# kngwyu/mujoco-maze

Measured on AMD Instinct MI355X. Metric: env-steps/sec (whole node), AntUMaze-v0, 4096 envs/GPU, higher is better.
Workload: dtype f32; 1 GPU; AntUMaze-v0, 4096 envs/GPU, frame_skip 5 x RK4, random actions uniform in the action box, auto-reset; 100 untimed settle steps + 5 warm-up steps before the timed window; envs_per_gpu=4096, obs_allgather=False, library=mujoco_maze_amd/csrc/libmazestep.so, lanes_per_env=library default, waves_per_block=1, bad_envs=0

## Files before the change

### mujoco_maze_amd/csrc/ant_newton_rows.h

```cpp
#pragma once
#include <type_traits>

#include "ant_dyn.h"
#include "mz_device.h"

namespace rows {

__host__ __device__ __forceinline__ constexpr int pos2dof(int p) { return (p & 3) < 2 ? 6 + 2 * (p >> 2) + (p & 1) : (p < 12 ? 2 * (p >> 2) + (p & 3) - 2 : p); }
__host__ __device__ __forceinline__ constexpr int dof2pos(int d) { return d < 6 ? 4 * (d >> 1) + 2 + (d & 1) : (d < 14 ? 4 * ((d - 6) >> 1) + ((d - 6) & 1) : d); }
static_assert(dof2pos(0) == 2 && dof2pos(5) == 11 && dof2pos(6) == 0 && dof2pos(13) == 13 && pos2dof(7) == 3 && pos2dof(9) == 11 && pos2dof(15) == 15, "row layout");

template <int P>
__device__ __forceinline__ float bcast(float x) {
  return __int_as_float(__builtin_amdgcn_mov_dpp(__float_as_int(x), 0x150 + P, 0xF, 0xF, true));
}
template <int P>
__device__ __forceinline__ int bcast_i(int x) { return __builtin_amdgcn_mov_dpp(x, 0x150 + P, 0xF, 0xF, true); }
__device__ __forceinline__ float rsum(float x) {
#pragma clang fp contract(off)
  x += __int_as_float(__builtin_amdgcn_mov_dpp(__float_as_int(x), 0xB1, 0xF, 0xF, true));
  x += __int_as_float(__builtin_amdgcn_mov_dpp(__float_as_int(x), 0x4E, 0xF, 0xF, true));
  x += __int_as_float(__builtin_amdgcn_mov_dpp(__float_as_int(x), 0x141, 0xF, 0xF, true));
  x += __int_as_float(__builtin_amdgcn_mov_dpp(__float_as_int(x), 0x140, 0xF, 0xF, true));
  return x;
}

#define MZ_DPP_TAIL " row_mask:0xf bank_mask:0xf\n\t"
#define MZ_MV_MUL(acc, k) "v_mul_f32_dpp %" #acc ", %[x], %[a" #k "] row_newbcast:" #k MZ_DPP_TAIL
#define MZ_MV_FMA(acc, k) "v_fmac_f32_dpp %" #acc ", %[x], %[a" #k "] row_newbcast:" #k MZ_DPP_TAIL

#define MZ_R3_OP(d, x, ctrl) "v_add_f32_dpp %[" #d "], %[" #x "], %[" #x "] " ctrl MZ_DPP_TAIL
#define MZ_R3_FIRST(ctrl) MZ_R3_OP(sa, a, ctrl) MZ_R3_OP(sb, b, ctrl) MZ_R3_OP(sc, c, ctrl)
#define MZ_R3_STEP(ctrl) MZ_R3_OP(sa, sa, ctrl) MZ_R3_OP(sb, sb, ctrl) MZ_R3_OP(sc, sc, ctrl)
#define MZ_R3_TREE MZ_R3_FIRST("quad_perm:[1,0,3,2]") MZ_R3_STEP("quad_perm:[2,3,0,1]") MZ_R3_STEP("row_half_mirror") MZ_R3_STEP("row_mirror")
__device__ __forceinline__ void rsum3(float a, float b, float c, float& sa, float& sb, float& sc) {
  asm("s_nop 1\n\t" MZ_R3_TREE : [sa] "=&v"(sa), [sb] "=&v"(sb), [sc] "=&v"(sc) : [a] "v"(a), [b] "v"(b), [c] "v"(c));
}
__device__ __forceinline__ void rsum3_q1(float a, float b, float c, float& sa, float& sb, float& sc, float& qa, float& qb, float& qc) {
  asm("s_nop 1\n\t" MZ_R3_OP(qa, a, "quad_perm:[1,1,1,1]") MZ_R3_OP(qb, b, "quad_perm:[1,1,1,1]") MZ_R3_OP(qc, c, "quad_perm:[1,1,1,1]") MZ_R3_TREE
      : [sa] "=&v"(sa), [sb] "=&v"(sb), [sc] "=&v"(sc), [qa] "=&v"(qa), [qb] "=&v"(qb), [qc] "=&v"(qc) : [a] "v"(a), [b] "v"(b), [c] "v"(c));
}

#define MZ_R2_FIRST(ctrl) "v_add_f32_dpp %0, %2, %2 " ctrl MZ_DPP_TAIL "v_add_f32_dpp %1, %3, %3 " ctrl MZ_DPP_TAIL
#define MZ_R2_STEP(ctrl) "s_nop 0\n\tv_add_f32_dpp %0, %0, %0 " ctrl MZ_DPP_TAIL "v_add_f32_dpp %1, %1, %1 " ctrl MZ_DPP_TAIL
__device__ __forceinline__ void rsum2(float a, float b, float& sa, float& sb) {
  asm("s_nop 1\n\t" MZ_R2_FIRST("quad_perm:[1,0,3,2]") MZ_R2_STEP("quad_perm:[2,3,0,1]") MZ_R2_STEP("row_half_mirror") MZ_R2_STEP("row_mirror")
      : "=&v"(sa), "=&v"(sb) : "v"(a), "v"(b));
}
#define MZ_R3_MUL "v_mul_f32 %[sa], %[a], %[x]\n\tv_mul_f32 %[sb], %[b], %[x]\n\tv_mul_f32 %[sc], %[c], %[x]\n\t"
__device__ __forceinline__ void rsum3_scaled(float a, float b, float c, float x, float& sa, float& sb, float& sc) {
  asm(MZ_R3_MUL MZ_R3_STEP("quad_perm:[1,0,3,2]") MZ_R3_STEP("quad_perm:[2,3,0,1]") MZ_R3_STEP("row_half_mirror") MZ_R3_STEP("row_mirror")
      : [sa] "=&v"(sa), [sb] "=&v"(sb), [sc] "=&v"(sc) : [a] "v"(a), [b] "v"(b), [c] "v"(c), [x] "v"(x));
}

__device__ __forceinline__ float matvec(const float (&A)[14], float x) {
  float s0, s1, s2;
  asm("s_nop 1\n\t" MZ_MV_MUL(0, 0) MZ_MV_MUL(1, 1) MZ_MV_MUL(2, 2) MZ_MV_FMA(0, 3) MZ_MV_FMA(1, 4) MZ_MV_FMA(2, 5) MZ_MV_FMA(0, 6) MZ_MV_FMA(1, 7)
      MZ_MV_FMA(2, 8) MZ_MV_FMA(0, 9) MZ_MV_FMA(1, 10) MZ_MV_FMA(2, 11) MZ_MV_FMA(0, 12) MZ_MV_FMA(1, 13)
      : "=&v"(s0), "=&v"(s1), "=&v"(s2)
      : [x] "v"(x), [a0] "v"(A[0]), [a1] "v"(A[1]), [a2] "v"(A[2]), [a3] "v"(A[3]), [a4] "v"(A[4]), [a5] "v"(A[5]), [a6] "v"(A[6]), [a7] "v"(A[7]),
        [a8] "v"(A[8]), [a9] "v"(A[9]), [a10] "v"(A[10]), [a11] "v"(A[11]), [a12] "v"(A[12]), [a13] "v"(A[13]));
  return (s0 + s1) + s2;
}
__device__ __forceinline__ float matvec(const float (&A)[16], float x) {
  float s0, s1, s2;
  asm("s_nop 1\n\t" MZ_MV_MUL(0, 0) MZ_MV_MUL(1, 1) MZ_MV_MUL(2, 2) MZ_MV_FMA(0, 3) MZ_MV_FMA(1, 4) MZ_MV_FMA(2, 5) MZ_MV_FMA(0, 6) MZ_MV_FMA(1, 7)
      MZ_MV_FMA(2, 8) MZ_MV_FMA(0, 9) MZ_MV_FMA(1, 10) MZ_MV_FMA(2, 11) MZ_MV_FMA(0, 12) MZ_MV_FMA(1, 13) MZ_MV_FMA(2, 14) MZ_MV_FMA(0, 15)
      : "=&v"(s0), "=&v"(s1), "=&v"(s2)
      : [x] "v"(x), [a0] "v"(A[0]), [a1] "v"(A[1]), [a2] "v"(A[2]), [a3] "v"(A[3]), [a4] "v"(A[4]), [a5] "v"(A[5]), [a6] "v"(A[6]), [a7] "v"(A[7]),
        [a8] "v"(A[8]), [a9] "v"(A[9]), [a10] "v"(A[10]), [a11] "v"(A[11]), [a12] "v"(A[12]), [a13] "v"(A[13]), [a14] "v"(A[14]), [a15] "v"(A[15]));
  return (s0 + s1) + s2;
}

#define MZ_EL(i) "v_fmac_f32_dpp %" #i ", %" #i ", %[li] row_newbcast:%[p]" MZ_DPP_TAIL
#define MZ_EL_IN [li] "v"(nli), [p] "n"(P)
template <int P> __device__ __forceinline__ void elim(float nli, float& b) { asm("s_nop 1\n\t" MZ_EL(0) : "+v"(b) : MZ_EL_IN); }
template <int P> __device__ __forceinline__ void elim(float nli, float& b, float& h0) { asm("s_nop 1\n\t" MZ_EL(0) MZ_EL(1) : "+v"(b), "+v"(h0) : MZ_EL_IN); }
template <int P> __device__ __forceinline__ void elim(float nli, float& b, float& h0, float& h1) {
  asm("s_nop 1\n\t" MZ_EL(0) MZ_EL(1) MZ_EL(2) : "+v"(b), "+v"(h0), "+v"(h1) : MZ_EL_IN);
}
template <int P> __device__ __forceinline__ void elim(float nli, float& b, float& h0, float& h1, float& h2) {
  asm("s_nop 1\n\t" MZ_EL(0) MZ_EL(1) MZ_EL(2) MZ_EL(3) : "+v"(b), "+v"(h0), "+v"(h1), "+v"(h2) : MZ_EL_IN);
}
template <int P> __device__ __forceinline__ void elim(float nli, float& b, float& h0, float& h1, float& h2, float& h3) {
  asm("s_nop 1\n\t" MZ_EL(0) MZ_EL(1) MZ_EL(2) MZ_EL(3) MZ_EL(4) : "+v"(b), "+v"(h0), "+v"(h1), "+v"(h2), "+v"(h3) : MZ_EL_IN);
}
template <int P> __device__ __forceinline__ void elim(float nli, float& b, float& h0, float& h1, float& h2, float& h3, float& h4) {
  asm("s_nop 1\n\t" MZ_EL(0) MZ_EL(1) MZ_EL(2) MZ_EL(3) MZ_EL(4) MZ_EL(5) : "+v"(b), "+v"(h0), "+v"(h1), "+v"(h2), "+v"(h3), "+v"(h4) : MZ_EL_IN);
}
template <int P> __device__ __forceinline__ void elim(float nli, float& b, float& h0, float& h1, float& h2, float& h3, float& h4, float& h5) {
  asm("s_nop 1\n\t" MZ_EL(0) MZ_EL(1) MZ_EL(2) MZ_EL(3) MZ_EL(4) MZ_EL(5) MZ_EL(6)
      : "+v"(b), "+v"(h0), "+v"(h1), "+v"(h2), "+v"(h3), "+v"(h4), "+v"(h5) : MZ_EL_IN);
}
template <int P> __device__ __forceinline__ void elim(float nli, float& b, float& h0, float& h1, float& h2, float& h3, float& h4, float& h5, float& h6) {
  asm("s_nop 1\n\t" MZ_EL(0) MZ_EL(1) MZ_EL(2) MZ_EL(3) MZ_EL(4) MZ_EL(5) MZ_EL(6) MZ_EL(7)
      : "+v"(b), "+v"(h0), "+v"(h1), "+v"(h2), "+v"(h3), "+v"(h4), "+v"(h5), "+v"(h6) : MZ_EL_IN);
}
template <int P> __device__ __forceinline__ void elim(float nli, float& b, float& h0, float& h1, float& h2, float& h3, float& h4, float& h5, float& h6, float& h7) {
  asm("s_nop 1\n\t" MZ_EL(0) MZ_EL(1) MZ_EL(2) MZ_EL(3) MZ_EL(4) MZ_EL(5) MZ_EL(6) MZ_EL(7) MZ_EL(8)
      : "+v"(b), "+v"(h0), "+v"(h1), "+v"(h2), "+v"(h3), "+v"(h4), "+v"(h5), "+v"(h6), "+v"(h7) : MZ_EL_IN);
}
template <int P> __device__ __forceinline__ void elim(float nli, float& b, float& h0, float& h1, float& h2, float& h3, float& h4, float& h5, float& h6, float& h7, float& h8) {
  asm("s_nop 1\n\t" MZ_EL(0) MZ_EL(1) MZ_EL(2) MZ_EL(3) MZ_EL(4) MZ_EL(5) MZ_EL(6) MZ_EL(7) MZ_EL(8) MZ_EL(9)
      : "+v"(b), "+v"(h0), "+v"(h1), "+v"(h2), "+v"(h3), "+v"(h4), "+v"(h5), "+v"(h6), "+v"(h7), "+v"(h8) : MZ_EL_IN);
}

#define MZ_FA_MUL(o, c, j) "v_mul_f32_dpp %" #o ", %[" #c "], %[" #j "] row_newbcast:%[p]" MZ_DPP_TAIL
#define MZ_FA_FMA(o, c, j) "v_fmac_f32_dpp %" #o ", %[" #c "], %[" #j "] row_newbcast:%[p]" MZ_DPP_TAIL
template <int P>
__device__ __forceinline__ void fold_t(const float (&cg)[8], float j0, float j1, float j2, float& t, float& t0, float& t1, float& t2) {
  asm("s_nop 1\n\t" MZ_FA_MUL(0, c0, j0) MZ_FA_MUL(1, c3, j0) MZ_FA_MUL(2, c4, j0) MZ_FA_MUL(3, c5, j0) MZ_FA_FMA(0, c1, j1) MZ_FA_FMA(1, c4, j1)
      MZ_FA_FMA(2, c6, j1) MZ_FA_FMA(3, c7, j2) MZ_FA_FMA(0, c2, j2) MZ_FA_FMA(1, c5, j2)
      : "=&v"(t), "=&v"(t0), "=&v"(t1), "=&v"(t2)
      : [c0] "v"(cg[0]), [c1] "v"(cg[1]), [c2] "v"(cg[2]), [c3] "v"(cg[3]), [c4] "v"(cg[4]), [c5] "v"(cg[5]), [c6] "v"(cg[6]), [c7] "v"(cg[7]),
        [j0] "v"(j0), [j1] "v"(j1), [j2] "v"(j2), [p] "n"(P));
}
template <int P>
__device__ __forceinline__ float fold_g(float g0, float g1, float g2, float j0, float j1, float j2) {
  float a0, a1, a2;
  asm("s_nop 1\n\t" MZ_FA_MUL(0, c0, j0) MZ_FA_MUL(1, c1, j1) MZ_FA_MUL(2, c2, j2)
      : "=&v"(a0), "=&v"(a1), "=&v"(a2) : [c0] "v"(g0), [c1] "v"(g1), [c2] "v"(g2), [j0] "v"(j0), [j1] "v"(j1), [j2] "v"(j2), [p] "n"(P));
  return (a0 + a1) + a2;
}
#define MZ_FH(k, j, t) "v_fmac_f32_dpp %" #k ", %[" #j "], %[" #t "] row_newbcast:" #k MZ_DPP_TAIL
#define MZ_FH14(j, t) MZ_FH(0, j, t) MZ_FH(1, j, t) MZ_FH(2, j, t) MZ_FH(3, j, t) MZ_FH(4, j, t) MZ_FH(5, j, t) MZ_FH(6, j, t) MZ_FH(7, j, t) \
                      MZ_FH(8, j, t) MZ_FH(9, j, t) MZ_FH(10, j, t) MZ_FH(11, j, t) MZ_FH(12, j, t) MZ_FH(13, j, t)
#define MZ_FH16(j, t) MZ_FH14(j, t) MZ_FH(14, j, t) MZ_FH(15, j, t)
#define MZ_FH_IN [j0] "v"(j0), [j1] "v"(j1), [j2] "v"(j2), [t0] "v"(t0), [t1] "v"(t1), [t2] "v"(t2)
__device__ __forceinline__ void fold_h(float (&H)[14], float j0, float j1, float j2, float t0, float t1, float t2) {
  asm("s_nop 1\n\t" MZ_FH14(j0, t0) MZ_FH14(j1, t1) MZ_FH14(j2, t2)
      : "+v"(H[0]), "+v"(H[1]), "+v"(H[2]), "+v"(H[3]), "+v"(H[4]), "+v"(H[5]), "+v"(H[6]), "+v"(H[7]), "+v"(H[8]), "+v"(H[9]), "+v"(H[10]),
        "+v"(H[11]), "+v"(H[12]), "+v"(H[13])
      : MZ_FH_IN);
}
__device__ __forceinline__ void fold_h(float (&H)[16], float j0, float j1, float j2, float t0, float t1, float t2) {
  asm("s_nop 1\n\t" MZ_FH16(j0, t0) MZ_FH16(j1, t1) MZ_FH16(j2, t2)
      : "+v"(H[0]), "+v"(H[1]), "+v"(H[2]), "+v"(H[3]), "+v"(H[4]), "+v"(H[5]), "+v"(H[6]), "+v"(H[7]), "+v"(H[8]), "+v"(H[9]), "+v"(H[10]),
        "+v"(H[11]), "+v"(H[12]), "+v"(H[13]), "+v"(H[14]), "+v"(H[15])
      : MZ_FH_IN);
}

typedef float v16f __attribute__((ext_vector_type(16)));
__device__ __forceinline__ void mfma_operands_ready(float& t0, float& t1, float& t2) { asm("s_nop 3" : "+v"(t0), "+v"(t1), "+v"(t2)); }
__device__ __forceinline__ void fold_h_mfma(v16f& acc, float j0, float j1, float j2, float t0, float t1, float t2) {
  mfma_operands_ready(t0, t1, t2);
  acc = __builtin_amdgcn_mfma_f32_16x16x1f32(t0, j0, acc, 0, 0, 0);
  acc = __builtin_amdgcn_mfma_f32_16x16x1f32(t1, j1, acc, 0, 0, 0);
  acc = __builtin_amdgcn_mfma_f32_16x16x1f32(t2, j2, acc, 0, 0, 0);
}
__device__ __forceinline__ void mfma_rows(const v16f& acc, float (&out)[16]) {
  float G[4][4];
#pragma unroll
  for (int b = 0; b < 4; b++)
#pragma unroll
    for (int v = 0; v < 4; v++) G[b][v] = acc[4 * b + v];
#pragma unroll
  for (int v = 0; v < 4; v++) {
    auto r0 = __builtin_amdgcn_permlane32_swap(__float_as_int(G[0][v]), __float_as_int(G[2][v]), false, false);
    G[0][v] = __int_as_float(r0[0]); G[2][v] = __int_as_float(r0[1]);
    auto r1 = __builtin_amdgcn_permlane32_swap(__float_as_int(G[1][v]), __float_as_int(G[3][v]), false, false);
    G[1][v] = __int_as_float(r1[0]); G[3][v] = __int_as_float(r1[1]);
  }
#pragma unroll
  for (int v = 0; v < 4; v++) {
    auto r0 = __builtin_amdgcn_permlane16_swap(__float_as_int(G[0][v]), __float_as_int(G[1][v]), false, false);
    G[0][v] = __int_as_float(r0[0]); G[1][v] = __int_as_float(r0[1]);
    auto r1 = __builtin_amdgcn_permlane16_swap(__float_as_int(G[2][v]), __float_as_int(G[3][v]), false, false);
    G[2][v] = __int_as_float(r1[0]); G[3][v] = __int_as_float(r1[1]);
  }
#pragma unroll
  for (int g = 0; g < 4; g++)
#pragma unroll
    for (int v = 0; v < 4; v++) out[4 * g + v] = G[g][v];
}

__device__ __forceinline__ float pivot_floor() { float t = 1e-30f; asm("" : "+v"(t)); return t; }
template <int P>
__device__ __forceinline__ float pivot_clamped(float h, float tiny) {
  float d;
  asm("s_nop 1\n\tv_max_f32_dpp %0, %1, %2 row_newbcast:%3 row_mask:0xf bank_mask:0xf" : "=&v"(d) : "v"(h), "v"(tiny), "n"(P));
  return d;
}

template <int P, int N, int... COLS>
__device__ __forceinline__ void pivot(int r, float tiny, float (&Hrow)[N], float& b, float& dinv, float (&mlt)[N]) {
  asm("" : "+v"(r));
  const float ri = 1.0f / pivot_clamped<P>(Hrow[P], tiny);
  const float nli = (r == P) ? 0.f : -(Hrow[P] * ri);
  elim<P>(nli, b, Hrow[COLS]...);
  dinv = (r == P) ? ri : dinv;
  mlt[P] = nli;
}

__device__ __forceinline__ float solve_rows(int r, float (&Hrow)[14], float b, float (&mlt)[14], float& dinv) {
  dinv = 0.f;
  const float tiny = pivot_floor();
  pivot<0, 14, 1, 2, 3, 6, 7, 10, 11>(r, tiny, Hrow, b, dinv, mlt);
  pivot<4, 14, 5, 2, 3, 6, 7, 10, 11>(r, tiny, Hrow, b, dinv, mlt);
  pivot<8, 14, 9, 2, 3, 6, 7, 10, 11>(r, tiny, Hrow, b, dinv, mlt);
  pivot<12, 14, 13, 2, 3, 6, 7, 10, 11>(r, tiny, Hrow, b, dinv, mlt);
  pivot<1, 14, 2, 3, 6, 7, 10, 11>(r, tiny, Hrow, b, dinv, mlt);
  pivot<5, 14, 2, 3, 6, 7, 10, 11>(r, tiny, Hrow, b, dinv, mlt);
  pivot<9, 14, 2, 3, 6, 7, 10, 11>(r, tiny, Hrow, b, dinv, mlt);
  pivot<13, 14, 2, 3, 6, 7, 10, 11>(r, tiny, Hrow, b, dinv, mlt);
  pivot<2, 14, 3, 6, 7, 10, 11>(r, tiny, Hrow, b, dinv, mlt);
  pivot<3, 14, 6, 7, 10, 11>(r, tiny, Hrow, b, dinv, mlt);
  pivot<6, 14, 7, 10, 11>(r, tiny, Hrow, b, dinv, mlt);
  pivot<7, 14, 10, 11>(r, tiny, Hrow, b, dinv, mlt);
  pivot<10, 14, 11>(r, tiny, Hrow, b, dinv, mlt);
  pivot<11, 14>(r, tiny, Hrow, b, dinv, mlt);
  return b * dinv;
}
__device__ __forceinline__ float solve_rows(int r, float (&Hrow)[14], float b) {
  float mlt[14], dinv;
  return solve_rows(r, Hrow, b, mlt, dinv);
}
__device__ __forceinline__ float solve_rows(int r, float (&Hrow)[16], float b, float (&mlt)[16], float& dinv) {
  dinv = 0.f;
  const float tiny = pivot_floor();
  pivot<0, 16, 1, 2, 3, 6, 7, 10, 11, 14, 15>(r, tiny, Hrow, b, dinv, mlt);
  pivot<4, 16, 5, 2, 3, 6, 7, 10, 11, 14, 15>(r, tiny, Hrow, b, dinv, mlt);
  pivot<8, 16, 9, 2, 3, 6, 7, 10, 11, 14, 15>(r, tiny, Hrow, b, dinv, mlt);
  pivot<12, 16, 13, 2, 3, 6, 7, 10, 11, 14, 15>(r, tiny, Hrow, b, dinv, mlt);
  pivot<1, 16, 2, 3, 6, 7, 10, 11, 14, 15>(r, tiny, Hrow, b, dinv, mlt);
  pivot<5, 16, 2, 3, 6, 7, 10, 11, 14, 15>(r, tiny, Hrow, b, dinv, mlt);
  pivot<9, 16, 2, 3, 6, 7, 10, 11, 14, 15>(r, tiny, Hrow, b, dinv, mlt);
  pivot<13, 16, 2, 3, 6, 7, 10, 11, 14, 15>(r, tiny, Hrow, b, dinv, mlt);
  pivot<14, 16, 15, 2, 3, 6, 7, 10, 11>(r, tiny, Hrow, b, dinv, mlt);
  pivot<15, 16, 2, 3, 6, 7, 10, 11>(r, tiny, Hrow, b, dinv, mlt);
  pivot<2, 16, 3, 6, 7, 10, 11>(r, tiny, Hrow, b, dinv, mlt);
  pivot<3, 16, 6, 7, 10, 11>(r, tiny, Hrow, b, dinv, mlt);
  pivot<6, 16, 7, 10, 11>(r, tiny, Hrow, b, dinv, mlt);
  pivot<7, 16, 10, 11>(r, tiny, Hrow, b, dinv, mlt);
  pivot<10, 16, 11>(r, tiny, Hrow, b, dinv, mlt);
  pivot<11, 16>(r, tiny, Hrow, b, dinv, mlt);
  return b * dinv;
}

__device__ __forceinline__ float solve_rows(int r, float (&Hrow)[16], float b) {
  float mlt[16], dinv;
  return solve_rows(r, Hrow, b, mlt, dinv);
}
template <int P>
__device__ __forceinline__ void repivot(float m, float& b) { elim<P>(m, b); }
__device__ __forceinline__ float resolve_rows(const float (&mlt)[16], float dinv, float b) {
  repivot<0>(mlt[0], b); repivot<4>(mlt[4], b); repivot<8>(mlt[8], b); repivot<12>(mlt[12], b);
  repivot<1>(mlt[1], b); repivot<5>(mlt[5], b); repivot<9>(mlt[9], b); repivot<13>(mlt[13], b);
  repivot<14>(mlt[14], b); repivot<15>(mlt[15], b);
  repivot<2>(mlt[2], b); repivot<3>(mlt[3], b); repivot<6>(mlt[6], b); repivot<7>(mlt[7], b); repivot<10>(mlt[10], b); repivot<11>(mlt[11], b);
  return b * dinv;
}
__device__ __forceinline__ float resolve_rows(const float (&mlt)[14], float dinv, float b) {
  repivot<0>(mlt[0], b); repivot<4>(mlt[4], b); repivot<8>(mlt[8], b); repivot<12>(mlt[12], b);
  repivot<1>(mlt[1], b); repivot<5>(mlt[5], b); repivot<9>(mlt[9], b); repivot<13>(mlt[13], b);
  repivot<2>(mlt[2], b); repivot<3>(mlt[3], b); repivot<6>(mlt[6], b); repivot<7>(mlt[7], b); repivot<10>(mlt[10], b); repivot<11>(mlt[11], b);
  return b * dinv;
}

#define MZ_D6_MUL(o, k) "v_mul_f32_dpp %" #o ", %[f" #k "], %[s" #k "] row_newbcast:%[q]" MZ_DPP_TAIL
#define MZ_D6_FMA(o, k) "v_fmac_f32_dpp %" #o ", %[f" #k "], %[s" #k "] row_newbcast:%[q]" MZ_DPP_TAIL
template <int Q>
__device__ __forceinline__ float dot6_from(const float (&F)[6], const float (&S)[6]) {
  float a0, a1, a2;
  asm("s_nop 1\n\t" MZ_D6_MUL(0, 0) MZ_D6_MUL(1, 1) MZ_D6_MUL(2, 2) MZ_D6_FMA(0, 3) MZ_D6_FMA(1, 4) MZ_D6_FMA(2, 5)
      : "=&v"(a0), "=&v"(a1), "=&v"(a2)
      : [f0] "v"(F[0]), [f1] "v"(F[1]), [f2] "v"(F[2]), [f3] "v"(F[3]), [f4] "v"(F[4]), [f5] "v"(F[5]), [s0] "v"(S[0]), [s1] "v"(S[1]), [s2] "v"(S[2]),
        [s3] "v"(S[3]), [s4] "v"(S[4]), [s5] "v"(S[5]), [q] "n"(Q));
  return (a0 + a1) + a2;
}
__device__ __forceinline__ float ceval(float D, float u0, float u1, float u2) {
  float r0 = u0 + u1, r1 = u0 - u1, r2 = u0 + u2, r3 = u0 - u2;
  float c = 0.f;
  if (r0 < 0.f) c += r0 * r0;
  if (r1 < 0.f) c += r1 * r1;
  if (r2 < 0.f) c += r2 * r2;
  if (r3 < 0.f) c += r3 * r3;
  return 0.5f * D * c;
}

__device__ __forceinline__ float bsel(int m, float a, float b) { return __int_as_float((__float_as_int(a) & m) | (__float_as_int(b) & ~m)); }

template <int NB>
__device__ __forceinline__ void contact_record(const AntDev& K, const float* pos, const float* n, float dist, int kind, const float* hint, int cls, int leg,
                                               const float* vb, const float* vblk, float tran, float* rec) {
  const int mk = -(int)(kind == 0);
  struct { float margin, mu, K, B; } P = {bsel(mk, K.floor.margin, K.wall.margin), bsel(mk, K.floor.mu, K.wall.mu), bsel(mk, K.floor.K, K.wall.K),
                                         bsel(mk, K.floor.B, K.wall.B)};
  float si[7];
#pragma unroll
  for (int k = 0; k < 7; k++) si[k] = bsel(mk, K.floor.solimp[k], K.wall.solimp[k]);
  float t1[3], t2[3];
  make_tangents(n, hint, t1, t2);
  const float sr = bsel(mk, 1.f, -1.f);
  float omi;
  const float imp = impedance_pair(si, fabsf(dist - P.margin), &omi);
  if (NB == 1 && kind == 2) tran += K.block_bw_tran;
  const float Rr = fmaxf(1e-15f, omi / imp * (tran + P.mu * P.mu * tran));
  rec[7] = 1.0f / (2.f * P.mu * P.mu * Rr);
  rec[15] = __int_as_float((leg < 0 ? 7 : leg) | (cls << 3) | ((NB == 1 && kind == 2) ? 64 : 0));
  rec[23] = 0.f;
#pragma unroll
  for (int a = 0; a < 3; a++) {
    const float sc = (a == 0 ? 1.f : P.mu) * sr;
    const float* dir = a == 0 ? n : (a == 1 ? t1 : t2);
    const float f[3] = {sc * dir[0], sc * dir[1], sc * dir[2]};
    float m[3];
    cross3f(m, pos, f);
    float* w = rec + 8 * a;
    w[0] = m[0]; w[1] = m[1]; w[2] = m[2]; w[3] = f[0]; w[4] = f[1]; w[5] = f[2];
    float vel = m[0] * vb[0] + m[1] * vb[1] + m[2] * vb[2] + f[0] * vb[3] + f[1] * vb[4] + f[2] * vb[5];
    if constexpr (NB == 1) {
      if (kind == 2) {
#pragma unroll
        for (int sl = 0; sl < 2; sl++) vel -= (K.block_axis[sl] == 0 ? f[0] : (K.block_axis[sl] == 1 ? f[1] : f[2])) * vblk[sl];
      }
    }
    float aref = -P.B * vel;
    if (a == 0) aref -= P.K * imp * (dist - P.margin);
    w[6] = aref;
  }
}

__device__ __forceinline__ void contact_raw_store(float* q, const float* pos, const float* n, float dist, int kind, const float* hint, int cls, int leg,
                                                  const float* vb, float tran) {
  float4* dst = reinterpret_cast<float4*>(q);
  dst[0] = make_float4(pos[0], pos[1], pos[2], n[0]);
  dst[1] = make_float4(n[1], n[2], dist, __int_as_float(kind | ((cls + 1) << 4) | ((leg + 1) << 8)));
  dst[2] = make_float4(hint[0], hint[1], hint[2], vb[0]);
  dst[3] = make_float4(vb[1], vb[2], vb[3], vb[4]);
  dst[4] = make_float4(vb[5], tran, 0.f, 0.f);
}
}

template <class S>
__device__ __forceinline__ float* wr_record(S& s, int c) { return &s.cJ[0][0][0] + 24 * c; }
template <class S>
__device__ __forceinline__ const float* wr_record(const S& s, int c) { return &s.cJ[0][0][0] + 24 * c; }

enum { LC_LO = 11, LC_HI = 12, LC_DOFW = 13 };
enum { LU_FLOORM = 14, LU_WALLM, LU_SCALE, LU_INVS, LU_TX, LU_TY, LU_HXY, LU_HZ, LU_CZ, LU_GRID, LU_ARM, LU_DAMP, LU_GZ, LU_TOL, LU_RTOL, LU_ISC,
       LU_ITERS, LU_LS, LU_N };
struct AntU {
  float floor_margin, wall_margin, scale, inv_scale_xy, tx, ty, half_xy, half_z, center_z;
  int rows, cols;
  bool elevated;
  float armature, damping, gz, tol, rtol, inv_scale;
  int max_iter, ls_iter, ls_fast_iters, ls_fast, trust_exact;
};
template <int G, bool PROF>
__device__ __forceinline__ AntU ant_u(const DevCtx<G, PROF>& cx, const AntDev& K) {
  const MazeDev& z = K.maze;
  if (cx.mfma)
    return {K.floor.margin, K.wall.margin, z.scale, 1.0f / z.scale, z.tx, z.ty, z.half_xy, z.half_z, z.center_z, z.rows, z.cols, z.elevated != 0,
            K.armature, K.damping, K.gz, K.tol, K.rtol, K.inv_scale, K.max_iter, K.ls_iter, K.ls_fast_iters, K.ls_fast, K.trust_exact};
  const int g = __float_as_int(cx.lc[LU_GRID]);
  const int a = __builtin_amdgcn_readfirstlane(__float_as_int(cx.lc[LU_ITERS])), b = __builtin_amdgcn_readfirstlane(__float_as_int(cx.lc[LU_LS]));
  return {cx.lc[LU_FLOORM], cx.lc[LU_WALLM], cx.lc[LU_SCALE], cx.lc[LU_INVS], cx.lc[LU_TX], cx.lc[LU_TY], cx.lc[LU_HXY], cx.lc[LU_HZ], cx.lc[LU_CZ],
          g & 255, (g >> 8) & 255, ((g >> 16) & 1) != 0, cx.lc[LU_ARM], cx.lc[LU_DAMP], cx.lc[LU_GZ], cx.lc[LU_TOL], cx.lc[LU_RTOL], cx.lc[LU_ISC],
          a, b & 1023, (b >> 10) & 1023, (b >> 20) & 1023, (b >> 30) & 1};
}
__device__ __forceinline__ float lu_hold(float x) { asm("" : "+v"(x)); return x; }
template <int G, bool PROF>
__device__ __forceinline__ void ant_limit_consts(const AntDev& K, DevCtx<G, PROF>& cx) {
  static_assert(LU_N <= DevCtx<G, PROF>::NLC, "DevCtx::lc too small");
  const int p = cx.l & 15, l = p >> 2, d = p & 1;
  cx.lc[LC_LO] = d ? K.ank_lo[l] : K.hip_lo; cx.lc[LC_HI] = d ? K.ank_hi[l] : K.hip_hi; cx.lc[LC_DOFW] = d ? K.dofw_ank : K.dofw_hip;
  if (cx.mfma) return;
  const MazeDev& z = K.maze;
  cx.lc[LU_FLOORM] = lu_hold(K.floor.margin); cx.lc[LU_WALLM] = lu_hold(K.wall.margin);
  cx.lc[LU_SCALE] = lu_hold(z.scale); cx.lc[LU_INVS] = lu_hold(1.0f / z.scale); cx.lc[LU_TX] = lu_hold(z.tx); cx.lc[LU_TY] = lu_hold(z.ty);
  cx.lc[LU_HXY] = lu_hold(z.half_xy); cx.lc[LU_HZ] = lu_hold(z.half_z); cx.lc[LU_CZ] = lu_hold(z.center_z);
  cx.lc[LU_GRID] = lu_hold(__int_as_float(z.rows | (z.cols << 8) | ((z.elevated ? 1 : 0) << 16)));
  cx.lc[LU_ARM] = lu_hold(K.armature); cx.lc[LU_DAMP] = lu_hold(K.damping); cx.lc[LU_GZ] = lu_hold(K.gz);
  cx.lc[LU_TOL] = lu_hold(K.tol); cx.lc[LU_RTOL] = lu_hold(K.rtol); cx.lc[LU_ISC] = lu_hold(K.inv_scale);
  auto c10 = [](int v) { return v < 0 ? 0 : (v > 1023 ? 1023 : v); };
  cx.lc[LU_ITERS] = lu_hold(__int_as_float(K.max_iter < 0 ? 0 : K.max_iter));
  cx.lc[LU_LS] = lu_hold(__int_as_float(c10(K.ls_iter) | (c10(K.ls_fast_iters) << 10) | (c10(K.ls_fast) << 20) | ((K.trust_exact ? 1 : 0) << 30)));
}

template <int NB>
__device__ __forceinline__ void block_rows_direct(const AntDev& K, const AntScratchCoreT<NB>& s, int c, float (&jb)[3][2], float (&ar)[3], float& Dout) {
  using D = AntDims<NB>;
  const int src = s.csrc[c];
  const float* q = src >= 0 ? con_stage<NB>(s, src) : &s.cY[c][0][0];
  const float n[3] = {q[3], q[4], q[5]}, dist = q[6];
  const int code = (int)q[7], kind = code & 15, other = (code >> 7) & 15;
  const float mult = (float)((code >> 11) + 1);
  const float v0 = s.qvel[14], v1 = s.qvel[15];
  if (kind == 6) {
    const float sg = n[0] + n[1] + n[2];
    jb[0][0] = other == 0 ? sg : 0.f; jb[0][1] = other == 1 ? sg : 0.f;
    jb[1][0] = jb[1][1] = jb[2][0] = jb[2][1] = 0.f;
    const float vel = sg * (other == 0 ? v0 : v1);
    float omi;
    const float imp = impedance_pair(K.blim_solimp, fabsf(dist - K.blim_margin), &omi);
    const float R = fmaxf(1e-15f, omi / imp * K.blim_w);
    Dout = 0.25f / R;
    ar[0] = -K.blim_B * vel - K.blim_K * imp * (dist - K.blim_margin); ar[1] = 0.f; ar[2] = 0.f;
    return;
  }
  const bool fl = kind == 3;
  struct { float margin, mu, K, B; } P = {fl ? K.floor.margin : K.wall.margin, fl ? K.floor.mu : K.wall.mu, fl ? K.floor.K : K.wall.K, fl ? K.floor.B : K.wall.B};
  float psi[7];
#pragma unroll
  for (int k = 0; k < 7; k++) { const float fv = K.floor.solimp[k], wv = K.wall.solimp[k]; psi[k] = fl ? fv : wv; }
  const float hint[3] = {0.f, 0.f, 0.f};
  float t1[3], t2[3];
  make_tangents(n, hint, t1, t2);
#pragma unroll
  for (int a = 0; a < 3; a++) {
    const float sc = a == 0 ? 1.f : P.mu;
    const float* dir = a == 0 ? n : (a == 1 ? t1 : t2);
#pragma unroll
    for (int sl = 0; sl < 2; sl++) jb[a][sl] = sc * (K.block_axis[sl] == 0 ? dir[0] : (K.block_axis[sl] == 1 ? dir[1] : dir[2]));
    ar[a] = -P.B * (jb[a][0] * v0 + jb[a][1] * v1);
  }
  float omi;
  const float imp = impedance_pair(psi, fabsf(dist - P.margin), &omi);
  const float tran = K.block_bw_tran;
  const float R = fmaxf(1e-15f, omi / imp * (tran + P.mu * P.mu * tran));
  Dout = mult / (2.f * P.mu * P.mu * R);
  ar[0] -= P.K * imp * (dist - P.margin);
  (void)sizeof(D);
}

#define MZ_IF_OWNER(c) if (true)
template <int NB, int G, bool PROF, bool WR = false, class SCR>
__device__ __forceinline__ float ant_solve_rows_core(const DevCtx<G, PROF>& cx, const AntDev& K, SCR& s, bool compare,
                                                    const float (&Mrow)[14 + 2 * NB], const float qfs, const float (&Sax)[6], const float hq, const float hv) {
  static_assert(G >= 16, "one DPP row per env at least");
  static_assert(NB <= 1, "one 16-lane row holds 14 dofs + one block's two slides");
  using namespace rows;
  using D = AntDims<NB>;
  constexpr int NR = 14 + 2 * NB;
  constexpr int NHC = D::NH;
  constexpr int BW = WR ? 16 : G;
  constexpr int MB = NB ? (WR ? 1 : (D::NC + G - 1) / G) : 0;
  constexpr int MA = NB ? 2 : 1;
  constexpr bool REFINE = NB == 1;
  const int r = cx.l & 15;
  const bool isdof = r < NR, ishinge = (r & 3) < 2 && r < 14;
  const int leg = r >> 2, d = r & 1;
  const int nB = NB ? s.nblkcon : 0;
  int nA = s.ncon - nB;
  if (nA > 16 * MA) { nA = 16 * MA; if (cx.l == 0) s.status |= MZ_STATUS_CONTACT_OVERFLOW; }
  if (NB && MB * BW < nB && cx.l == 0) s.status |= MZ_STATUS_CONTACT_OVERFLOW;
  auto bsum = [&](float x) { if constexpr (WR) return rsum(x); else return cx.gsum(x); };
  const int ncon = nA;
  const bool any2 = MA > 1 && cx.any(nA > 16);
  bool iscon[MA];
  int cr[MA], cl[MA];
#pragma unroll
  for (int m = 0; m < MA; m++) { iscon[m] = r + 16 * m < ncon; cr[m] = nB + (iscon[m] ? r + 16 * m : 0); cl[m] = (!WR && iscon[m]) ? s.cleg[cr[m]] : -1; }

  const int ri = isdof ? pos2dof(r) : 0;
  cx.tick(s, 12);
  float lsign = 0.f, lD = 0.f, laref = 0.f;
  if (ishinge) {
    const float q = hq, lo = cx.lc[LC_LO], hi = cx.lc[LC_HI];
    float pos = 0.f;
    if (q - lo < 0.f) { lsign = 1.f; pos = q - lo; }
    else if (hi - q < 0.f) { lsign = -1.f; pos = hi - q; }
    if (lsign != 0.f) {
      float omi;
      const float imp = impedance_pair(K.lim_solimp, fabsf(pos), &omi);
      const float R = fmaxf(1e-15f, omi / imp * cx.lc[LC_DOFW]);
      lD = 1.0f / R;
      laref = -K.lim_B * (lsign * hv) - K.lim_K * imp * pos;
    }
  }
  const bool has = s.ncon > 0 || cx.gany(lsign != 0.f);
  float qas = 0.f;
  if (compare || cx.any(!has)) {
    float Hq[NR];
#pragma unroll
    for (int k = 0; k < NR; k++) Hq[k] = Mrow[k];
    qas = solve_rows(r, Hq, qfs);
    if (isdof) s.qas[ri] = qas;
  }
  const float warm = isdof ? s.warm[ri] : 0.f;
  float cD[MA], ar[MA][3];
  float wr[MA][3][6];
  int wmeta[MA];
#pragma unroll
  for (int m = 0; m < MA; m++) wmeta[m] = 0;
  if constexpr (WR) {
#pragma unroll
    for (int m = 0; m < MA; m++) {
#pragma unroll
      for (int a = 0; a < 3; a++) {
#pragma unroll
        for (int k = 0; k < 6; k++) wr[m][a][k] = 0.f;
        ar[m][a] = 0.f;
      }
      cD[m] = 0.f;
      if (m == 1 && !any2) continue;
      const float4* q = reinterpret_cast<const float4*>(wr_record(s, cr[m]));
      float raw[20];
#pragma unroll
      for (int k = 0; k < 5; k++) { const float4 v4 = q[k]; raw[4 * k] = v4.x; raw[4 * k + 1] = v4.y; raw[4 * k + 2] = v4.z; raw[4 * k + 3] = v4.w; }
      const int rmeta = __float_as_int(raw[7]);
      const float vblk[2] = {NB == 1 ? s.qvel[14] : 0.f, NB == 1 ? s.qvel[14 + (NB == 1 ? 1 : 0)] : 0.f};
      float rec[24];
      contact_record<NB>(K, raw, raw + 3, raw[6], rmeta & 15, raw + 8, ((rmeta >> 4) & 15) - 1, ((rmeta >> 8) & 15) - 1, raw + 11, vblk, raw[17], rec);
      const int on = -(int)iscon[m];
#pragma unroll
      for (int a = 0; a < 3; a++) {
#pragma unroll
        for (int k = 0; k < 6; k++) wr[m][a][k] = __int_as_float(__float_as_int(rec[8 * a + k]) & on);
        ar[m][a] = __int_as_float(__float_as_int(rec[8 * a + 6]) & on);
      }
      cD[m] = __int_as_float(__float_as_int(rec[7]) & on);
      wmeta[m] = __float_as_int(rec[15]) & on;
    }
  } else {
#pragma unroll
    for (int m = 0; m < MA; m++) {
      cD[m] = iscon[m] ? s.cD[cr[m]] : 0.f;
#pragma unroll
      for (int a = 0; a < 3; a++) ar[m][a] = iscon[m] ? s.caref[cr[m]][a] : 0.f;
    }
  }
  float bj[MB ? MB : 1][3][2], bar[MB ? MB : 1][3], bD[MB ? MB : 1], bu[MB ? MB : 1][3], bv[MB ? MB : 1][3];
  if constexpr (NB == 1) {
#pragma unroll
    for (int m = 0; m < MB; m++) {
      const int c = (WR ? (cx.l & 15) : cx.l) + m * BW;
      const bool on = c < nB;
      bD[m] = 0.f;
#pragma unroll
      for (int a = 0; a < 3; a++) { bj[m][a][0] = 0.f; bj[m][a][1] = 0.f; bar[m][a] = 0.f; bu[m][a] = 0.f; bv[m][a] = 0.f; }
      if (on) block_rows_direct<NB>(K, s, c, bj[m], bar[m], bD[m]);
    }
  }

  auto each_contact = [&](auto&& f) {
    auto more = [&](int k) { return NB == 1 || cx.any(ncon > k); };
    if (cx.any(ncon > 0)) { f(std::integral_constant<int, 0>{});
    if (more(1)) { f(std::integral_constant<int, 1>{});
    if (more(2)) { f(std::integral_constant<int, 2>{});
    if (more(3)) { f(std::integral_constant<int, 3>{});
      if (cx.any(ncon > 4)) {
        f(std::integral_constant<int, 4>{}); f(std::integral_constant<int, 5>{});
        if (cx.any(ncon > 6)) { f(std::integral_constant<int, 6>{}); f(std::integral_constant<int, 7>{}); }
        if (cx.any(ncon > 8)) {
          f(std::integral_constant<int, 8>{}); f(std::integral_constant<int, 9>{}); f(std::integral_constant<int, 10>{}); f(std::integral_constant<int, 11>{});
          if (cx.any(ncon > 12)) { f(std::integral_constant<int, 12>{}); f(std::integral_constant<int, 13>{}); f(std::integral_constant<int, 14>{}); f(std::integral_constant<int, 15>{}); }
          if constexpr (MA > 1) {
            if (any2) {
              f(std::integral_constant<int, 16>{}); f(std::integral_constant<int, 17>{}); f(std::integral_constant<int, 18>{}); f(std::integral_constant<int, 19>{});
              if (cx.any(ncon > 20)) {
                f(std::integral_constant<int, 20>{}); f(std::integral_constant<int, 21>{}); f(std::integral_constant<int, 22>{}); f(std::integral_constant<int, 23>{});
                if (cx.any(ncon > 24)) {
                  f(std::integral_constant<int, 24>{}); f(std::integral_constant<int, 25>{}); f(std::integral_constant<int, 26>{}); f(std::integral_constant<int, 27>{});
                  f(std::integral_constant<int, 28>{}); f(std::integral_constant<int, 29>{}); f(std::integral_constant<int, 30>{}); f(std::integral_constant<int, 31>{});
                }
              }
            }
          }
        }
      }
    }}}}
  };
  constexpr int NJ = WR ? 16 : 16 * MA;
  float jown[NJ][3];
  auto wr_col = [&](auto Cc, float (&o)[3]) {
    constexpr int C = decltype(Cc)::value;
    const int mc = bcast_i<(C & 15)>(wmeta[C / 16]), lc = mc & 7, cc = (mc >> 3) & 7;
    const bool sees = C < ncon && (ishinge ? (leg == lc && (d == 0 ? cc >= 2 : cc == 3)) : (r < 12 || (NB == 1 && r >= 14 && (mc & 64) != 0)));
    const int on = -(int)sees;
#pragma unroll
    for (int a = 0; a < 3; a++) o[a] = __int_as_float(__float_as_int(dot6_from<(C & 15)>(wr[C / 16][a], Sax)) & on);
  };
  auto own_col = [&](auto Cc, float (&o)[3]) {
    constexpr int C = decltype(Cc)::value;
    if constexpr (WR && C >= 16) wr_col(Cc, o);
    else { o[0] = jown[C < NJ ? C : 0][0]; o[1] = jown[C < NJ ? C : 0][1]; o[2] = jown[C < NJ ? C : 0][2]; }
  };
  each_contact([&](auto Cc) {
    constexpr int C = decltype(Cc)::value;
    if constexpr (WR && C >= 16) return;
    else {
    jown[C][0] = jown[C][1] = jown[C][2] = 0.f;
    if constexpr (WR) {
      wr_col(Cc, jown[C]);
    } else
    if (C < ncon) {
      const int lc = s.cleg[nB + C];
      const int col = ishinge ? (leg == lc ? NHC + d : -1) : (r < 12 ? ri : ((NB == 1 && r >= 14 && r < 16) ? r - 8 : -1));
      if (col >= 0) { jown[C][0] = s.cJ[nB + C][0][col]; jown[C][1] = s.cJ[nB + C][1][col]; jown[C][2] = s.cJ[nB + C][2][col]; }
    }
    }
  });
  float Jf[MA][3][NR];
  if constexpr (!WR)
#pragma unroll
  for (int m = 0; m < MA; m++) {
#pragma unroll
    for (int a = 0; a < 3; a++)
#pragma unroll
      for (int k = 0; k < NR; k++) Jf[m][a][k] = 0.f;
    if (m == 1 && !any2) continue;
    if (iscon[m]) {
#pragma unroll
      for (int a = 0; a < 3; a++) {
        const float* Jr = s.cJ[cr[m]][a];
#pragma unroll
        for (int k = 0; k < 6; k++) Jf[m][a][dof2pos(k)] = Jr[k];
        if constexpr (NB == 1) { Jf[m][a][14] = Jr[6]; Jf[m][a][15] = Jr[7]; }
        const float jh = Jr[NHC], ja = Jr[NHC + 1];
#pragma unroll
        for (int l2 = 0; l2 < 4; l2++) { Jf[m][a][4 * l2] = cl[m] == l2 ? jh : 0.f; Jf[m][a][4 * l2 + 1] = cl[m] == l2 ? ja : 0.f; }
      }
    }
  }
  auto jdot3 = [&](float x, float (&o)[MA][3]) {
    if constexpr (WR) {
#pragma unroll
      for (int m = 0; m < MA; m++) o[m][0] = o[m][1] = o[m][2] = 0.f;
      each_contact([&](auto Cc) {
        constexpr int C = decltype(Cc)::value;
        {
          float jc[3];
          own_col(Cc, jc);
          float t0, t1, t2;
          rsum3_scaled(jc[0], jc[1], jc[2], x, t0, t1, t2);
          if (r == (C & 15)) { o[C / 16][0] = t0; o[C / 16][1] = t1; o[C / 16][2] = t2; }
        }
      });
    } else {
#pragma unroll
      for (int m = 0; m < MA; m++) {
        o[m][0] = o[m][1] = o[m][2] = 0.f;
        if (m == 1 && !any2) continue;
        o[m][0] = matvec(Jf[m][0], x); o[m][1] = matvec(Jf[m][1], x); o[m][2] = matvec(Jf[m][2], x);
      }
    }
  };
  auto bdot = [&](float b0, float b1, float (&o)[MB ? MB : 1][3]) {
#pragma unroll
    for (int m = 0; m < MB; m++)
#pragma unroll
      for (int a = 0; a < 3; a++) o[m][a] = bj[m][a][0] * b0 + bj[m][a][1] * b1;
  };

  float qacc = warm;
  if (compare) {
    const float dw = warm - qas;
    float cw = 0.5f * dw * matvec(Mrow, dw), cs = 0.f;
    float jw3[MA][3], jq3[MA][3];
    jdot3(warm, jw3);
    jdot3(qas, jq3);
#pragma unroll
    for (int m = 0; m < MA; m++)
      if (iscon[m]) {
        cw += ceval(cD[m], jw3[m][0] - ar[m][0], jw3[m][1] - ar[m][1], jw3[m][2] - ar[m][2]);
        cs += ceval(cD[m], jq3[m][0] - ar[m][0], jq3[m][1] - ar[m][1], jq3[m][2] - ar[m][2]);
      }
    if (lsign != 0.f) {
      const float jw = lsign * warm - laref, js = lsign * qas - laref;
      if (jw < 0.f) cw += 0.5f * lD * jw * jw;
      if (js < 0.f) cs += 0.5f * lD * js * js;
    }
    rsum2(cw, cs, cw, cs);
    if constexpr (NB == 1) {
      float bw[MB][3], bs[MB][3], cwb = 0.f, csb = 0.f;
      bdot(bcast<14>(warm), bcast<15>(warm), bw);
      bdot(bcast<14>(qas), bcast<15>(qas), bs);
#pragma unroll
      for (int m = 0; m < MB; m++) {
        cwb += ceval(bD[m], bw[m][0] - bar[m][0], bw[m][1] - bar[m][1], bw[m][2] - bar[m][2]);
        csb += ceval(bD[m], bs[m][0] - bar[m][0], bs[m][1] - bar[m][1], bs[m][2] - bar[m][2]);
      }
      cw += bsum(cwb); cs += bsum(csb);
    }
    qacc = cw < cs ? warm : qas;
  }
  if (!has) qacc = qas;
  cx.tick(s, 4);
  bool done = !has;
  int it = 0;
  float Mx = 0.f, ljar = 0.f, lact = 0.f, u[MA][3], v[MA][3];
#pragma unroll
  for (int m = 0; m < MA; m++) { u[m][0] = u[m][1] = u[m][2] = 0.f; v[m][0] = v[m][1] = v[m][2] = 0.f; }
  if (cx.any(!done)) {
    Mx = matvec(Mrow, qacc) - qfs;
    jdot3(qacc, u);
#pragma unroll
    for (int m = 0; m < MA; m++) { u[m][0] -= ar[m][0]; u[m][1] -= ar[m][1]; u[m][2] -= ar[m][2]; }
    if (lsign != 0.f) { ljar = lsign * qacc - laref; lact = ljar < 0.f ? lD : 0.f; }
    if constexpr (NB == 1) {
      bdot(bcast<14>(qacc), bcast<15>(qacc), bu);
#pragma unroll
      for (int m = 0; m < MB; m++)
#pragma unroll
        for (int a = 0; a < 3; a++) bu[m][a] -= bar[m][a];
    }
  }
  while (cx.any(!done) && it < ant_u(cx, K).max_iter) {
    float mycg[MA][8];
#pragma unroll
    for (int m = 0; m < MA; m++) {
#pragma unroll
      for (int k = 0; k < 8; k++) mycg[m][k] = 0.f;
      if (m == 1 && !any2) continue;
      MZ_IF_OWNER(iscon[m]) {
        const float u0 = u[m][0], u1 = u[m][1], u2 = u[m][2], Dm = cD[m];
        const float r0 = u0 + u1, r1 = u0 - u1, r2 = u0 + u2, r3 = u0 - u2;
        const float a0 = r0 < 0.f ? 1.f : 0.f, a1 = r1 < 0.f ? 1.f : 0.f, a2 = r2 < 0.f ? 1.f : 0.f, a3 = r3 < 0.f ? 1.f : 0.f;
        mycg[m][0] = Dm * (a0 * r0 + a1 * r1 + a2 * r2 + a3 * r3); mycg[m][1] = Dm * (a0 * r0 - a1 * r1); mycg[m][2] = Dm * (a2 * r2 - a3 * r3);
        mycg[m][3] = Dm * (a0 + a1 + a2 + a3); mycg[m][4] = Dm * (a0 - a1); mycg[m][5] = Dm * (a2 - a3); mycg[m][6] = Dm * (a0 + a1); mycg[m][7] = Dm * (a2 + a3);
      }
    }
    float bg0 = 0.f, bg1 = 0.f, bga0 = 0.f, bga1 = 0.f, bh00 = 0.f, bh01 = 0.f, bh11 = 0.f;
    if constexpr (NB == 1) {
#pragma unroll
      for (int m = 0; m < MB; m++) {
        const float x0 = bu[m][0], x1 = bu[m][1], x2 = bu[m][2], Dm = bD[m];
        const float r0 = x0 + x1, r1 = x0 - x1, r2 = x0 + x2, r3 = x0 - x2;
        const float a0 = r0 < 0.f ? 1.f : 0.f, a1 = r1 < 0.f ? 1.f : 0.f, a2 = r2 < 0.f ? 1.f : 0.f, a3 = r3 < 0.f ? 1.f : 0.f;
        const float g0 = Dm * (a0 * r0 + a1 * r1 + a2 * r2 + a3 * r3), g1 = Dm * (a0 * r0 - a1 * r1), g2 = Dm * (a2 * r2 - a3 * r3);
        const float W0 = Dm * (a0 + a1 + a2 + a3), W1 = Dm * (a0 - a1), W2 = Dm * (a2 - a3), W3 = Dm * (a0 + a1), W4 = Dm * (a2 + a3);
#pragma unroll
        for (int c = 0; c < 2; c++) {
          const float j0 = bj[m][0][c], j1 = bj[m][1][c], j2 = bj[m][2][c];
          const float t = j0 * g0 + j1 * g1 + j2 * g2;
          if (c == 0) { bg0 += t; bga0 += fabsf(t); } else { bg1 += t; bga1 += fabsf(t); }
          const float t0 = j0 * W0 + j1 * W1 + j2 * W2, t1 = j0 * W1 + j1 * W3, t2 = j0 * W2 + j2 * W4;
          if (c == 0) { bh00 += t0 * j0 + t1 * j1 + t2 * j2; bh01 += t0 * bj[m][0][1] + t1 * bj[m][1][1] + t2 * bj[m][2][1]; }
          else bh11 += t0 * j0 + t1 * j1 + t2 * j2;
        }
      }
      if constexpr (WR) {
        rsum3(bg0, bg1, bh00, bg0, bg1, bh00); rsum2(bga0, bga1, bga0, bga1); rsum2(bh01, bh11, bh01, bh11);
      } else {
        bg0 = bsum(bg0); bg1 = bsum(bg1); bga0 = bsum(bga0); bga1 = bsum(bga1);
        bh00 = bsum(bh00); bh01 = bsum(bh01); bh11 = bsum(bh11);
      }
    }
    float Hrow[NR];
#pragma unroll
    for (int k = 0; k < NR; k++) Hrow[k] = Mrow[k];
    float g = Mx, ga = fabsf(Mx);
    if (cx.mfma) {
     if (cx.any(ncon > 0)) {
      v16f hacc = {0.f, 0.f, 0.f, 0.f, 0.f, 0.f, 0.f, 0.f, 0.f, 0.f, 0.f, 0.f, 0.f, 0.f, 0.f, 0.f};
      each_contact([&](auto Cc) {
        constexpr int C = decltype(Cc)::value;
        float t, t0, t1, t2;
        float jc[3];
        own_col(Cc, jc);
        fold_t<(C & 15)>(mycg[C / 16], jc[0], jc[1], jc[2], t, t0, t1, t2);
        g += t; ga += fabsf(t);
        fold_h_mfma(hacc, jc[0], jc[1], jc[2], t0, t1, t2);
      });
      float hc[16];
      mfma_rows(hacc, hc);
#pragma unroll
      for (int k = 0; k < NR; k++) Hrow[k] += hc[k];
     }
    } else
    each_contact([&](auto Cc) {
      constexpr int C = decltype(Cc)::value;
      {
        float t, t0, t1, t2;
        float jc[3];
        own_col(Cc, jc);
        fold_t<(C & 15)>(mycg[C / 16], jc[0], jc[1], jc[2], t, t0, t1, t2);
        g += t; ga += fabsf(t);
        fold_h(Hrow, jc[0], jc[1], jc[2], t0, t1, t2);
      }
    });
    if constexpr (NB == 1) {
      if (r == 14) { g += bg0; ga += bga0; Hrow[14] += bh00; Hrow[15] += bh01; }
      if (r == 15) { g += bg1; ga += bga1; Hrow[14] += bh01; Hrow[15] += bh11; }
    }
    MZ_IF_OWNER(lsign != 0.f) { const float t = lsign * lact * ljar; g += t; ga += fabsf(t); }
#pragma unroll
    for (int k = 0; k < 14; k++)
      if ((k & 3) < 2) Hrow[k] += (r == k) ? lact : 0.f;
    if (!isdof) { g = 0.f; ga = 0.f; }
    float gnorm = 0.f, anorm = 0.f;
    if (it > 0) {
      rsum2(g * g, ga * ga, gnorm, anorm);
      gnorm = sqrtf(gnorm); anorm = sqrtf(anorm);
      if (!done && (ant_u(cx, K).inv_scale * gnorm < ant_u(cx, K).tol || gnorm <= ant_u(cx, K).rtol * anorm)) done = true;
    }
    if (!cx.any(!done)) { cx.tick(s, 5); break; }
    cx.tick(s, 5);
    float mlt[NR], dinv;
    const float search = solve_rows(r, Hrow, -g, mlt, dinv);
    cx.tick(s, 6);
    jdot3(search, v);
    const float ljv = lsign * search;
    bool changed = false;
#pragma unroll
    for (int m = 0; m < MA; m++)
      if (m == 0 || any2) MZ_IF_OWNER(iscon[m]) {
        const float u0 = u[m][0], u1 = u[m][1], u2 = u[m][2], w0 = u0 + v[m][0], w1 = u1 + v[m][1], w2 = u2 + v[m][2];
        changed = changed || ((u0 + u1 < 0.f) != (w0 + w1 < 0.f)) || ((u0 - u1 < 0.f) != (w0 - w1 < 0.f)) || ((u0 + u2 < 0.f) != (w0 + w2 < 0.f)) ||
                  ((u0 - u2 < 0.f) != (w0 - w2 < 0.f));
      }
    MZ_IF_OWNER(lsign != 0.f) changed = changed || ((ljar < 0.f) != (ljar + ljv < 0.f));
    if constexpr (NB == 1) {
      bdot(bcast<14>(search), bcast<15>(search), bv);
#pragma unroll
      for (int m = 0; m < MB; m++) {
        const float x0 = bu[m][0], x1 = bu[m][1], x2 = bu[m][2], w0 = x0 + bv[m][0], w1 = x1 + bv[m][1], w2 = x2 + bv[m][2];
        changed = changed || ((x0 + x1 < 0.f) != (w0 + w1 < 0.f)) || ((x0 - x1 < 0.f) != (w0 - w1 < 0.f)) || ((x0 + x2 < 0.f) != (w0 + w2 < 0.f)) ||
                  ((x0 - x2 < 0.f) != (w0 - w2 < 0.f));
      }
    }
    changed = cx.gany(changed);
    float alpha = 1.f, Ms = 0.f, sn = 1.f, qn = 0.f;
    const bool exact = !changed;
    if (changed) {
      Ms = matvec(Mrow, search);
      float p1, p2;
      rsum2(search * Mx, search * Ms, p1, p2);
      rsum2(isdof ? search * search : 0.f, isdof ? qacc * qacc : 0.f, sn, qn);
      float lo = 0.f, hi = -1.f, prev_d2 = -1.f;
      const int ls_max = it < ant_u(cx, K).ls_fast_iters ? ant_u(cx, K).ls_fast : ant_u(cx, K).ls_iter;
      for (int ls = 0; ls < ls_max; ls++) {
        float d1 = 0.f, d2 = 0.f;
#pragma unroll
        for (int m = 0; m < MA; m++)
          if (m == 0 || any2) MZ_IF_OWNER(iscon[m]) {
            const float v0 = v[m][0], v1 = v[m][1], v2 = v[m][2], Dm = cD[m];
            const float x0 = u[m][0] + alpha * v0, x1 = u[m][1] + alpha * v1, x2 = u[m][2] + alpha * v2;
            float rr, vv;
            rr = x0 + x1; vv = v0 + v1; if (rr < 0.f) { d1 += Dm * rr * vv; d2 += Dm * vv * vv; }
            rr = x0 - x1; vv = v0 - v1; if (rr < 0.f) { d1 += Dm * rr * vv; d2 += Dm * vv * vv; }
            rr = x0 + x2; vv = v0 + v2; if (rr < 0.f) { d1 += Dm * rr * vv; d2 += Dm * vv * vv; }
            rr = x0 - x2; vv = v0 - v2; if (rr < 0.f) { d1 += Dm * rr * vv; d2 += Dm * vv * vv; }
          }
        MZ_IF_OWNER(lsign != 0.f) { const float rr = ljar + alpha * ljv; if (rr < 0.f) { d1 += lD * rr * ljv; d2 += lD * ljv * ljv; } }
        if constexpr (NB != 1 || !WR) {
          rsum2(d1, d2, d1, d2);
          d1 = d1 + p1 + alpha * p2;
          d2 = d2 + p2;
        }
        if constexpr (NB == 1) {
          float e1 = 0.f, e2 = 0.f;
#pragma unroll
          for (int m = 0; m < MB; m++) {
            const float y0 = bv[m][0], y1 = bv[m][1], y2 = bv[m][2], Dm = bD[m];
            const float x0 = bu[m][0] + alpha * y0, x1 = bu[m][1] + alpha * y1, x2 = bu[m][2] + alpha * y2;
            float rr, vv;
            rr = x0 + x1; vv = y0 + y1; if (rr < 0.f) { e1 += Dm * rr * vv; e2 += Dm * vv * vv; }
            rr = x0 - x1; vv = y0 - y1; if (rr < 0.f) { e1 += Dm * rr * vv; e2 += Dm * vv * vv; }
            rr = x0 + x2; vv = y0 + y2; if (rr < 0.f) { e1 += Dm * rr * vv; e2 += Dm * vv * vv; }
            rr = x0 - x2; vv = y0 - y2; if (rr < 0.f) { e1 += Dm * rr * vv; e2 += Dm * vv * vv; }
          }
          if constexpr (WR) { rsum2(d1 + e1, d2 + e2, d1, d2); d1 = d1 + p1 + alpha * p2; d2 = d2 + p2; }
          else { d1 += cx.gsum(e1); d2 += cx.gsum(e2); }
        }
        if (d2 == prev_d2) break;
        prev_d2 = d2;
        if (d1 < 0.f) lo = alpha; else hi = alpha;
        float next = alpha - d1 / d2;
        if (hi >= 0.f && !(next > lo && next < hi)) next = 0.5f * (lo + hi);
        if (!(next > 0.f)) next = hi >= 0.f ? 0.5f * (lo + hi) : 0.f;
        if (fabsf(next - alpha) <= 1e-7f * fabsf(next)) { alpha = next; break; }
        alpha = next;
      }
    }
    if (done) alpha = 0.f;
    if (alpha != 0.f) {
      qacc += alpha * search;
      if (changed) {
        Mx += alpha * Ms;
#pragma unroll
        for (int m = 0; m < MA; m++) { u[m][0] += alpha * v[m][0]; u[m][1] += alpha * v[m][1]; u[m][2] += alpha * v[m][2]; }
        MZ_IF_OWNER(lsign != 0.f) { ljar += alpha * ljv; lact = ljar < 0.f ? lD : 0.f; }
        if constexpr (NB == 1) {
#pragma unroll
          for (int m = 0; m < MB; m++)
#pragma unroll
            for (int a = 0; a < 3; a++) bu[m][a] += alpha * bv[m][a];
        }
      }
    }
    if constexpr (REFINE) {
      if (cx.any(exact && !done)) {
        const float Ms2 = changed ? Ms : matvec(Mrow, search);
        float g2 = Mx + Ms2;
        float cg2[MA][3];
#pragma unroll
        for (int m = 0; m < MA; m++) {
          cg2[m][0] = cg2[m][1] = cg2[m][2] = 0.f;
          if (m == 1 && !any2) continue;
          const float u0 = u[m][0] + v[m][0], u1 = u[m][1] + v[m][1], u2 = u[m][2] + v[m][2], Dm = cD[m];
          const float r0 = u0 + u1, r1 = u0 - u1, r2 = u0 + u2, r3 = u0 - u2;
          const float a0 = r0 < 0.f ? r0 : 0.f, a1 = r1 < 0.f ? r1 : 0.f, a2 = r2 < 0.f ? r2 : 0.f, a3 = r3 < 0.f ? r3 : 0.f;
          cg2[m][0] = Dm * (a0 + a1 + a2 + a3); cg2[m][1] = Dm * (a0 - a1); cg2[m][2] = Dm * (a2 - a3);
        }
        each_contact([&](auto Cc) {
          constexpr int C = decltype(Cc)::value;
          float jc[3];
          own_col(Cc, jc);
          g2 += fold_g<(C & 15)>(cg2[C / 16][0], cg2[C / 16][1], cg2[C / 16][2], jc[0], jc[1], jc[2]);
        });
        {
          const float lj2 = ljar + ljv;
          g2 += lsign * (lj2 < 0.f ? lD : 0.f) * lj2;
        }
        if constexpr (NB == 1) {
          float c0 = 0.f, c1 = 0.f;
#pragma unroll
          for (int m = 0; m < MB; m++) {
            const float x0 = bu[m][0] + bv[m][0], x1 = bu[m][1] + bv[m][1], x2 = bu[m][2] + bv[m][2], Dm = bD[m];
            const float r0 = x0 + x1, r1 = x0 - x1, r2 = x0 + x2, r3 = x0 - x2;
            const float a0 = r0 < 0.f ? r0 : 0.f, a1 = r1 < 0.f ? r1 : 0.f, a2 = r2 < 0.f ? r2 : 0.f, a3 = r3 < 0.f ? r3 : 0.f;
            const float g0 = Dm * (a0 + a1 + a2 + a3), g1 = Dm * (a0 - a1), gg2 = Dm * (a2 - a3);
            c0 += bj[m][0][0] * g0 + bj[m][1][0] * g1 + bj[m][2][0] * gg2;
            c1 += bj[m][0][1] * g0 + bj[m][1][1] * g1 + bj[m][2][1] * gg2;
          }
          if constexpr (WR) rsum2(c0, c1, c0, c1); else { c0 = bsum(c0); c1 = bsum(c1); }
          if (r == 14) g2 += c0;
          if (r == 15) g2 += c1;
        }
        if (!isdof) g2 = 0.f;
        const float corr = resolve_rows(mlt, dinv, -g2);
        if (exact && !done) qacc += corr;
      }
    }
    if (exact && ant_u(cx, K).trust_exact) done = true;
    if (changed && alpha * alpha * sn <= MZ_NEWTON_STALL * MZ_NEWTON_STALL * qn) done = true;
    cx.tick(s, 7);
    it++;
  }
  if (isdof) s.qacc[ri] = qacc;
  if (cx.l == 0) {
    s.iters = it;
    if (it >= ant_u(cx, K).max_iter && !done) s.status |= MZ_STATUS_SOLVER_MAXITER;
    if constexpr (PROF) s.prof[15] += (unsigned)it;
  }
  cx.sync();
  cx.tick(s, 8);
  return qacc;
}
```

Measured before the change: 18.07 million env-steps/s.

## Fuse Newton solver DPP asm blocks and do Gauss-Jordan elimination in place

Rewrites the row-parallel Newton solver's hand-written DPP assembly. Hessian fold_t and fold_h are merged into one asm block. The pivot chain becomes a single in-place Gauss-Jordan asm sequence that keeps the multipliers in Hrow instead of a separate mlt array. Two rsum2 reductions are merged into one rsum4, and the three dot6 calls into one dot6x3. The aim is to cut s_nop wait states, asm boundaries and register pressure, at the cost of fragile hand-scheduled hazard handling and reuse of Hrow as multiplier storage.

After: 18.80 million env-steps/s, median of 6. 1.04x the previous value.

```diff
diff --git a/mujoco_maze_amd/csrc/ant_newton_rows.h b/mujoco_maze_amd/csrc/ant_newton_rows.h
--- a/mujoco_maze_amd/csrc/ant_newton_rows.h
+++ b/mujoco_maze_amd/csrc/ant_newton_rows.h
@@ -26,6 +26,13 @@
 }
 
 #define MZ_DPP_TAIL " row_mask:0xf bank_mask:0xf\n\t"
+#define MZ_ASM_W(W, body, ...)                                       \
+  do {                                                               \
+    static_assert(W >= 0 && W <= 2, "opening wait states: 0, 1, 2"); \
+    if constexpr (W == 0) asm(body __VA_ARGS__);                     \
+    else if constexpr (W == 1) asm("s_nop 0\n\t" body __VA_ARGS__);  \
+    else asm("s_nop 1\n\t" body __VA_ARGS__);                        \
+  } while (0)
 #define MZ_MV_MUL(acc, k) "v_mul_f32_dpp %" #acc ", %[x], %[a" #k "] row_newbcast:" #k MZ_DPP_TAIL
 #define MZ_MV_FMA(acc, k) "v_fmac_f32_dpp %" #acc ", %[x], %[a" #k "] row_newbcast:" #k MZ_DPP_TAIL
 
@@ -33,19 +40,34 @@
 #define MZ_R3_FIRST(ctrl) MZ_R3_OP(sa, a, ctrl) MZ_R3_OP(sb, b, ctrl) MZ_R3_OP(sc, c, ctrl)
 #define MZ_R3_STEP(ctrl) MZ_R3_OP(sa, sa, ctrl) MZ_R3_OP(sb, sb, ctrl) MZ_R3_OP(sc, sc, ctrl)
 #define MZ_R3_TREE MZ_R3_FIRST("quad_perm:[1,0,3,2]") MZ_R3_STEP("quad_perm:[2,3,0,1]") MZ_R3_STEP("row_half_mirror") MZ_R3_STEP("row_mirror")
+template <int W = 2>
 __device__ __forceinline__ void rsum3(float a, float b, float c, float& sa, float& sb, float& sc) {
-  asm("s_nop 1\n\t" MZ_R3_TREE : [sa] "=&v"(sa), [sb] "=&v"(sb), [sc] "=&v"(sc) : [a] "v"(a), [b] "v"(b), [c] "v"(c));
-}
+  MZ_ASM_W(W, MZ_R3_TREE, : [sa] "=&v"(sa), [sb] "=&v"(sb), [sc] "=&v"(sc) : [a] "v"(a), [b] "v"(b), [c] "v"(c));
+}
+template <int W = 2>
 __device__ __forceinline__ void rsum3_q1(float a, float b, float c, float& sa, float& sb, float& sc, float& qa, float& qb, float& qc) {
-  asm("s_nop 1\n\t" MZ_R3_OP(qa, a, "quad_perm:[1,1,1,1]") MZ_R3_OP(qb, b, "quad_perm:[1,1,1,1]") MZ_R3_OP(qc, c, "quad_perm:[1,1,1,1]") MZ_R3_TREE
-      : [sa] "=&v"(sa), [sb] "=&v"(sb), [sc] "=&v"(sc), [qa] "=&v"(qa), [qb] "=&v"(qb), [qc] "=&v"(qc) : [a] "v"(a), [b] "v"(b), [c] "v"(c));
+  MZ_ASM_W(W, MZ_R3_OP(qa, a, "quad_perm:[1,1,1,1]") MZ_R3_OP(qb, b, "quad_perm:[1,1,1,1]") MZ_R3_OP(qc, c, "quad_perm:[1,1,1,1]") MZ_R3_TREE,
+           : [sa] "=&v"(sa), [sb] "=&v"(sb), [sc] "=&v"(sc), [qa] "=&v"(qa), [qb] "=&v"(qb), [qc] "=&v"(qc) : [a] "v"(a), [b] "v"(b), [c] "v"(c));
 }
 
 #define MZ_R2_FIRST(ctrl) "v_add_f32_dpp %0, %2, %2 " ctrl MZ_DPP_TAIL "v_add_f32_dpp %1, %3, %3 " ctrl MZ_DPP_TAIL
 #define MZ_R2_STEP(ctrl) "s_nop 0\n\tv_add_f32_dpp %0, %0, %0 " ctrl MZ_DPP_TAIL "v_add_f32_dpp %1, %1, %1 " ctrl MZ_DPP_TAIL
+template <int W = 2>
 __device__ __forceinline__ void rsum2(float a, float b, float& sa, float& sb) {
-  asm("s_nop 1\n\t" MZ_R2_FIRST("quad_perm:[1,0,3,2]") MZ_R2_STEP("quad_perm:[2,3,0,1]") MZ_R2_STEP("row_half_mirror") MZ_R2_STEP("row_mirror")
+  MZ_ASM_W(W, MZ_R2_FIRST("quad_perm:[1,0,3,2]") MZ_R2_STEP("quad_perm:[2,3,0,1]") MZ_R2_STEP("row_half_mirror") MZ_R2_STEP("row_mirror"),
+           : "=&v"(sa), "=&v"(sb) : "v"(a), "v"(b));
+}
+__device__ __forceinline__ void rsum2_sq(float a, float b, float& sa, float& sb) {
+  asm("v_mul_f32 %0, %2, %2\n\tv_mul_f32 %1, %3, %3\n\t" MZ_R2_STEP("quad_perm:[1,0,3,2]") MZ_R2_STEP("quad_perm:[2,3,0,1]") MZ_R2_STEP("row_half_mirror")
+      MZ_R2_STEP("row_mirror")
       : "=&v"(sa), "=&v"(sb) : "v"(a), "v"(b));
+}
+#define MZ_R4_FIRST(ctrl) MZ_R3_FIRST(ctrl) MZ_R3_OP(sd, d, ctrl)
+#define MZ_R4_STEP(ctrl) MZ_R3_STEP(ctrl) MZ_R3_OP(sd, sd, ctrl)
+template <int W = 2>
+__device__ __forceinline__ void rsum4(float a, float b, float c, float d, float& sa, float& sb, float& sc, float& sd) {
+  MZ_ASM_W(W, MZ_R4_FIRST("quad_perm:[1,0,3,2]") MZ_R4_STEP("quad_perm:[2,3,0,1]") MZ_R4_STEP("row_half_mirror") MZ_R4_STEP("row_mirror"),
+           : [sa] "=&v"(sa), [sb] "=&v"(sb), [sc] "=&v"(sc), [sd] "=&v"(sd) : [a] "v"(a), [b] "v"(b), [c] "v"(c), [d] "v"(d));
 }
 #define MZ_R3_MUL "v_mul_f32 %[sa], %[a], %[x]\n\tv_mul_f32 %[sb], %[b], %[x]\n\tv_mul_f32 %[sc], %[c], %[x]\n\t"
 __device__ __forceinline__ void rsum3_scaled(float a, float b, float c, float x, float& sa, float& sb, float& sc) {
@@ -53,91 +75,65 @@
       : [sa] "=&v"(sa), [sb] "=&v"(sb), [sc] "=&v"(sc) : [a] "v"(a), [b] "v"(b), [c] "v"(c), [x] "v"(x));
 }
 
+template <int W = 2>
 __device__ __forceinline__ float matvec(const float (&A)[14], float x) {
   float s0, s1, s2;
-  asm("s_nop 1\n\t" MZ_MV_MUL(0, 0) MZ_MV_MUL(1, 1) MZ_MV_MUL(2, 2) MZ_MV_FMA(0, 3) MZ_MV_FMA(1, 4) MZ_MV_FMA(2, 5) MZ_MV_FMA(0, 6) MZ_MV_FMA(1, 7)
-      MZ_MV_FMA(2, 8) MZ_MV_FMA(0, 9) MZ_MV_FMA(1, 10) MZ_MV_FMA(2, 11) MZ_MV_FMA(0, 12) MZ_MV_FMA(1, 13)
+  MZ_ASM_W(W, MZ_MV_MUL(0, 0) MZ_MV_MUL(1, 1) MZ_MV_MUL(2, 2) MZ_MV_FMA(0, 3) MZ_MV_FMA(1, 4) MZ_MV_FMA(2, 5) MZ_MV_FMA(0, 6) MZ_MV_FMA(1, 7)
+      MZ_MV_FMA(2, 8) MZ_MV_FMA(0, 9) MZ_MV_FMA(1, 10) MZ_MV_FMA(2, 11) MZ_MV_FMA(0, 12) MZ_MV_FMA(1, 13),
       : "=&v"(s0), "=&v"(s1), "=&v"(s2)
       : [x] "v"(x), [a0] "v"(A[0]), [a1] "v"(A[1]), [a2] "v"(A[2]), [a3] "v"(A[3]), [a4] "v"(A[4]), [a5] "v"(A[5]), [a6] "v"(A[6]), [a7] "v"(A[7]),
         [a8] "v"(A[8]), [a9] "v"(A[9]), [a10] "v"(A[10]), [a11] "v"(A[11]), [a12] "v"(A[12]), [a13] "v"(A[13]));
   return (s0 + s1) + s2;
 }
+template <int W = 2>
 __device__ __forceinline__ float matvec(const float (&A)[16], float x) {
   float s0, s1, s2;
-  asm("s_nop 1\n\t" MZ_MV_MUL(0, 0) MZ_MV_MUL(1, 1) MZ_MV_MUL(2, 2) MZ_MV_FMA(0, 3) MZ_MV_FMA(1, 4) MZ_MV_FMA(2, 5) MZ_MV_FMA(0, 6) MZ_MV_FMA(1, 7)
-      MZ_MV_FMA(2, 8) MZ_MV_FMA(0, 9) MZ_MV_FMA(1, 10) MZ_MV_FMA(2, 11) MZ_MV_FMA(0, 12) MZ_MV_FMA(1, 13) MZ_MV_FMA(2, 14) MZ_MV_FMA(0, 15)
+  MZ_ASM_W(W, MZ_MV_MUL(0, 0) MZ_MV_MUL(1, 1) MZ_MV_MUL(2, 2) MZ_MV_FMA(0, 3) MZ_MV_FMA(1, 4) MZ_MV_FMA(2, 5) MZ_MV_FMA(0, 6) MZ_MV_FMA(1, 7)
+      MZ_MV_FMA(2, 8) MZ_MV_FMA(0, 9) MZ_MV_FMA(1, 10) MZ_MV_FMA(2, 11) MZ_MV_FMA(0, 12) MZ_MV_FMA(1, 13) MZ_MV_FMA(2, 14) MZ_MV_FMA(0, 15),
       : "=&v"(s0), "=&v"(s1), "=&v"(s2)
       : [x] "v"(x), [a0] "v"(A[0]), [a1] "v"(A[1]), [a2] "v"(A[2]), [a3] "v"(A[3]), [a4] "v"(A[4]), [a5] "v"(A[5]), [a6] "v"(A[6]), [a7] "v"(A[7]),
         [a8] "v"(A[8]), [a9] "v"(A[9]), [a10] "v"(A[10]), [a11] "v"(A[11]), [a12] "v"(A[12]), [a13] "v"(A[13]), [a14] "v"(A[14]), [a15] "v"(A[15]));
   return (s0 + s1) + s2;
 }
 
-#define MZ_EL(i) "v_fmac_f32_dpp %" #i ", %" #i ", %[li] row_newbcast:%[p]" MZ_DPP_TAIL
-#define MZ_EL_IN [li] "v"(nli), [p] "n"(P)
-template <int P> __device__ __forceinline__ void elim(float nli, float& b) { asm("s_nop 1\n\t" MZ_EL(0) : "+v"(b) : MZ_EL_IN); }
-template <int P> __device__ __forceinline__ void elim(float nli, float& b, float& h0) { asm("s_nop 1\n\t" MZ_EL(0) MZ_EL(1) : "+v"(b), "+v"(h0) : MZ_EL_IN); }
-template <int P> __device__ __forceinline__ void elim(float nli, float& b, float& h0, float& h1) {
-  asm("s_nop 1\n\t" MZ_EL(0) MZ_EL(1) MZ_EL(2) : "+v"(b), "+v"(h0), "+v"(h1) : MZ_EL_IN);
-}
-template <int P> __device__ __forceinline__ void elim(float nli, float& b, float& h0, float& h1, float& h2) {
-  asm("s_nop 1\n\t" MZ_EL(0) MZ_EL(1) MZ_EL(2) MZ_EL(3) : "+v"(b), "+v"(h0), "+v"(h1), "+v"(h2) : MZ_EL_IN);
-}
-template <int P> __device__ __forceinline__ void elim(float nli, float& b, float& h0, float& h1, float& h2, float& h3) {
-  asm("s_nop 1\n\t" MZ_EL(0) MZ_EL(1) MZ_EL(2) MZ_EL(3) MZ_EL(4) : "+v"(b), "+v"(h0), "+v"(h1), "+v"(h2), "+v"(h3) : MZ_EL_IN);
-}
-template <int P> __device__ __forceinline__ void elim(float nli, float& b, float& h0, float& h1, float& h2, float& h3, float& h4) {
-  asm("s_nop 1\n\t" MZ_EL(0) MZ_EL(1) MZ_EL(2) MZ_EL(3) MZ_EL(4) MZ_EL(5) : "+v"(b), "+v"(h0), "+v"(h1), "+v"(h2), "+v"(h3), "+v"(h4) : MZ_EL_IN);
-}
-template <int P> __device__ __forceinline__ void elim(float nli, float& b, float& h0, float& h1, float& h2, float& h3, float& h4, float& h5) {
-  asm("s_nop 1\n\t" MZ_EL(0) MZ_EL(1) MZ_EL(2) MZ_EL(3) MZ_EL(4) MZ_EL(5) MZ_EL(6)
-      : "+v"(b), "+v"(h0), "+v"(h1), "+v"(h2), "+v"(h3), "+v"(h4), "+v"(h5) : MZ_EL_IN);
-}
-template <int P> __device__ __forceinline__ void elim(float nli, float& b, float& h0, float& h1, float& h2, float& h3, float& h4, float& h5, float& h6) {
-  asm("s_nop 1\n\t" MZ_EL(0) MZ_EL(1) MZ_EL(2) MZ_EL(3) MZ_EL(4) MZ_EL(5) MZ_EL(6) MZ_EL(7)
-      : "+v"(b), "+v"(h0), "+v"(h1), "+v"(h2), "+v"(h3), "+v"(h4), "+v"(h5), "+v"(h6) : MZ_EL_IN);
-}
-template <int P> __device__ __forceinline__ void elim(float nli, float& b, float& h0, float& h1, float& h2, float& h3, float& h4, float& h5, float& h6, float& h7) {
-  asm("s_nop 1\n\t" MZ_EL(0) MZ_EL(1) MZ_EL(2) MZ_EL(3) MZ_EL(4) MZ_EL(5) MZ_EL(6) MZ_EL(7) MZ_EL(8)
-      : "+v"(b), "+v"(h0), "+v"(h1), "+v"(h2), "+v"(h3), "+v"(h4), "+v"(h5), "+v"(h6), "+v"(h7) : MZ_EL_IN);
-}
-template <int P> __device__ __forceinline__ void elim(float nli, float& b, float& h0, float& h1, float& h2, float& h3, float& h4, float& h5, float& h6, float& h7, float& h8) {
-  asm("s_nop 1\n\t" MZ_EL(0) MZ_EL(1) MZ_EL(2) MZ_EL(3) MZ_EL(4) MZ_EL(5) MZ_EL(6) MZ_EL(7) MZ_EL(8) MZ_EL(9)
-      : "+v"(b), "+v"(h0), "+v"(h1), "+v"(h2), "+v"(h3), "+v"(h4), "+v"(h5), "+v"(h6), "+v"(h7), "+v"(h8) : MZ_EL_IN);
-}
 
 #define MZ_FA_MUL(o, c, j) "v_mul_f32_dpp %" #o ", %[" #c "], %[" #j "] row_newbcast:%[p]" MZ_DPP_TAIL
 #define MZ_FA_FMA(o, c, j) "v_fmac_f32_dpp %" #o ", %[" #c "], %[" #j "] row_newbcast:%[p]" MZ_DPP_TAIL
-template <int P>
+#define MZ_FT(t, t0, t1, t2)                                                                                                        \
+  MZ_FA_MUL(t0, c3, j0) MZ_FA_MUL(t, c0, j0) MZ_FA_MUL(t1, c4, j0) MZ_FA_FMA(t0, c4, j1) MZ_FA_FMA(t, c1, j1) MZ_FA_MUL(t2, c5, j0) \
+  MZ_FA_FMA(t0, c5, j2) MZ_FA_FMA(t, c2, j2) MZ_FA_FMA(t1, c6, j1) MZ_FA_FMA(t2, c7, j2)
+#define MZ_FT_IN                                                                                                                             \
+  [c0] "v"(cg[0]), [c1] "v"(cg[1]), [c2] "v"(cg[2]), [c3] "v"(cg[3]), [c4] "v"(cg[4]), [c5] "v"(cg[5]), [c6] "v"(cg[6]), [c7] "v"(cg[7]), \
+      [j0] "v"(j0), [j1] "v"(j1), [j2] "v"(j2), [p] "n"(P)
+template <int P, int W = 2>
 __device__ __forceinline__ void fold_t(const float (&cg)[8], float j0, float j1, float j2, float& t, float& t0, float& t1, float& t2) {
-  asm("s_nop 1\n\t" MZ_FA_MUL(0, c0, j0) MZ_FA_MUL(1, c3, j0) MZ_FA_MUL(2, c4, j0) MZ_FA_MUL(3, c5, j0) MZ_FA_FMA(0, c1, j1) MZ_FA_FMA(1, c4, j1)
-      MZ_FA_FMA(2, c6, j1) MZ_FA_FMA(3, c7, j2) MZ_FA_FMA(0, c2, j2) MZ_FA_FMA(1, c5, j2)
-      : "=&v"(t), "=&v"(t0), "=&v"(t1), "=&v"(t2)
-      : [c0] "v"(cg[0]), [c1] "v"(cg[1]), [c2] "v"(cg[2]), [c3] "v"(cg[3]), [c4] "v"(cg[4]), [c5] "v"(cg[5]), [c6] "v"(cg[6]), [c7] "v"(cg[7]),
-        [j0] "v"(j0), [j1] "v"(j1), [j2] "v"(j2), [p] "n"(P));
-}
-template <int P>
+  MZ_ASM_W(W, MZ_FT(0, 1, 2, 3), : "=&v"(t), "=&v"(t0), "=&v"(t1), "=&v"(t2) : MZ_FT_IN);
+}
+template <int P, int W = 2>
 __device__ __forceinline__ float fold_g(float g0, float g1, float g2, float j0, float j1, float j2) {
   float a0, a1, a2;
-  asm("s_nop 1\n\t" MZ_FA_MUL(0, c0, j0) MZ_FA_MUL(1, c1, j1) MZ_FA_MUL(2, c2, j2)
+  MZ_ASM_W(W, MZ_FA_MUL(0, c0, j0) MZ_FA_MUL(1, c1, j1) MZ_FA_MUL(2, c2, j2),
       : "=&v"(a0), "=&v"(a1), "=&v"(a2) : [c0] "v"(g0), [c1] "v"(g1), [c2] "v"(g2), [j0] "v"(j0), [j1] "v"(j1), [j2] "v"(j2), [p] "n"(P));
   return (a0 + a1) + a2;
 }
-#define MZ_FH(k, j, t) "v_fmac_f32_dpp %" #k ", %[" #j "], %[" #t "] row_newbcast:" #k MZ_DPP_TAIL
-#define MZ_FH14(j, t) MZ_FH(0, j, t) MZ_FH(1, j, t) MZ_FH(2, j, t) MZ_FH(3, j, t) MZ_FH(4, j, t) MZ_FH(5, j, t) MZ_FH(6, j, t) MZ_FH(7, j, t) \
-                      MZ_FH(8, j, t) MZ_FH(9, j, t) MZ_FH(10, j, t) MZ_FH(11, j, t) MZ_FH(12, j, t) MZ_FH(13, j, t)
-#define MZ_FH16(j, t) MZ_FH14(j, t) MZ_FH(14, j, t) MZ_FH(15, j, t)
-#define MZ_FH_IN [j0] "v"(j0), [j1] "v"(j1), [j2] "v"(j2), [t0] "v"(t0), [t1] "v"(t1), [t2] "v"(t2)
-__device__ __forceinline__ void fold_h(float (&H)[14], float j0, float j1, float j2, float t0, float t1, float t2) {
-  asm("s_nop 1\n\t" MZ_FH14(j0, t0) MZ_FH14(j1, t1) MZ_FH14(j2, t2)
-      : "+v"(H[0]), "+v"(H[1]), "+v"(H[2]), "+v"(H[3]), "+v"(H[4]), "+v"(H[5]), "+v"(H[6]), "+v"(H[7]), "+v"(H[8]), "+v"(H[9]), "+v"(H[10]),
-        "+v"(H[11]), "+v"(H[12]), "+v"(H[13])
-      : MZ_FH_IN);
-}
-__device__ __forceinline__ void fold_h(float (&H)[16], float j0, float j1, float j2, float t0, float t1, float t2) {
-  asm("s_nop 1\n\t" MZ_FH16(j0, t0) MZ_FH16(j1, t1) MZ_FH16(j2, t2)
-      : "+v"(H[0]), "+v"(H[1]), "+v"(H[2]), "+v"(H[3]), "+v"(H[4]), "+v"(H[5]), "+v"(H[6]), "+v"(H[7]), "+v"(H[8]), "+v"(H[9]), "+v"(H[10]),
-        "+v"(H[11]), "+v"(H[12]), "+v"(H[13]), "+v"(H[14]), "+v"(H[15])
-      : MZ_FH_IN);
+#define MZ_FTH(k, j, t) "v_fmac_f32_dpp %[h" #k "], %[" #j "], %[" #t "] row_newbcast:" #k MZ_DPP_TAIL
+#define MZ_FTH14(j, t) MZ_FTH(0, j, t) MZ_FTH(1, j, t) MZ_FTH(2, j, t) MZ_FTH(3, j, t) MZ_FTH(4, j, t) MZ_FTH(5, j, t) MZ_FTH(6, j, t) MZ_FTH(7, j, t) \
+                       MZ_FTH(8, j, t) MZ_FTH(9, j, t) MZ_FTH(10, j, t) MZ_FTH(11, j, t) MZ_FTH(12, j, t) MZ_FTH(13, j, t)
+#define MZ_FTH16(j, t) MZ_FTH14(j, t) MZ_FTH(14, j, t) MZ_FTH(15, j, t)
+#define MZ_FTH_OUT14                                                                                                                              \
+  [t] "=&v"(t), [t0] "=&v"(t0), [t1] "=&v"(t1), [t2] "=&v"(t2), [h0] "+v"(H[0]), [h1] "+v"(H[1]), [h2] "+v"(H[2]), [h3] "+v"(H[3]), [h4] "+v"(H[4]), \
+      [h5] "+v"(H[5]), [h6] "+v"(H[6]), [h7] "+v"(H[7]), [h8] "+v"(H[8]), [h9] "+v"(H[9]), [h10] "+v"(H[10]), [h11] "+v"(H[11]), [h12] "+v"(H[12]), [h13] "+v"(H[13])
+template <int P, int W = 2>
+__device__ __forceinline__ float fold_th(float (&H)[14], const float (&cg)[8], float j0, float j1, float j2) {
+  float t, t0, t1, t2;
+  MZ_ASM_W(W, MZ_FT([t], [t0], [t1], [t2]) MZ_FTH14(j0, t0) MZ_FTH14(j1, t1) MZ_FTH14(j2, t2), : MZ_FTH_OUT14 : MZ_FT_IN);
+  return t;
+}
+template <int P, int W = 2>
+__device__ __forceinline__ float fold_th(float (&H)[16], const float (&cg)[8], float j0, float j1, float j2) {
+  float t, t0, t1, t2;
+  MZ_ASM_W(W, MZ_FT([t], [t0], [t1], [t2]) MZ_FTH16(j0, t0) MZ_FTH16(j1, t1) MZ_FTH16(j2, t2), : MZ_FTH_OUT14, [h14] "+v"(H[14]), [h15] "+v"(H[15]) : MZ_FT_IN);
+  return t;
 }
 
 typedef float v16f __attribute__((ext_vector_type(16)));
@@ -174,99 +170,123 @@
     for (int v = 0; v < 4; v++) out[4 * g + v] = G[g][v];
 }
 
-__device__ __forceinline__ float pivot_floor() { float t = 1e-30f; asm("" : "+v"(t)); return t; }
-template <int P>
-__device__ __forceinline__ float pivot_clamped(float h, float tiny) {
-  float d;
-  asm("s_nop 1\n\tv_max_f32_dpp %0, %1, %2 row_newbcast:%3 row_mask:0xf bank_mask:0xf" : "=&v"(d) : "v"(h), "v"(tiny), "n"(P));
-  return d;
-}
-
-template <int P, int N, int... COLS>
-__device__ __forceinline__ void pivot(int r, float tiny, float (&Hrow)[N], float& b, float& dinv, float (&mlt)[N]) {
-  asm("" : "+v"(r));
-  const float ri = 1.0f / pivot_clamped<P>(Hrow[P], tiny);
-  const float nli = (r == P) ? 0.f : -(Hrow[P] * ri);
-  elim<P>(nli, b, Hrow[COLS]...);
-  dinv = (r == P) ? ri : dinv;
-  mlt[P] = nli;
-}
-
-__device__ __forceinline__ float solve_rows(int r, float (&Hrow)[14], float b, float (&mlt)[14], float& dinv) {
+typedef unsigned long long lanemask_t;
+#define MZ_GJ_CMP(m, p) "v_cmp_eq_u32_e64 %[" #m "], " #p ", %[r]\n\t"
+#define MZ_GJ_GAP "s_nop 0\n\t"
+#define MZ_GJ_B(p) "v_fmac_f32_dpp %[b], %[b], %[h" #p "] row_newbcast:" #p MZ_DPP_TAIL
+#define MZ_GJ_E(k, p) "v_fmac_f32_dpp %[h" #k "], %[h" #k "], %[h" #p "] row_newbcast:" #p MZ_DPP_TAIL
+#define MZ_GJ_PIVOT(p, m, slot, el)                                                      \
+  "v_max_f32_dpp %[ri], %[h" #p "], %[tiny] row_newbcast:" #p MZ_DPP_TAIL                \
+  "v_rcp_f32_e32 %[ri], %[ri]\n\t" slot "v_mul_f32_e64 %[h" #p "], %[h" #p "], -%[ri]\n\t" \
+  "v_cndmask_b32_e64 %[h" #p "], %[h" #p "], 0, %[" #m "]\n\t"                             \
+  "v_cndmask_b32_e64 %[dinv], %[dinv], %[ri], %[" #m "]\n\t"                               \
+  "s_nop 0\n\t" el
+#define MZ_GJ_HINGE(p, pn, rk, rn, el)                                                                                    \
+  MZ_GJ_CMP(mb, p) "v_mul_f32_e64 %[h" #p "], %[h" #p "], -%[" #rk "]\n\t"                                                 \
+  "v_max_f32_dpp %[" #rn "], %[h" #pn "], %[tiny] row_newbcast:" #pn MZ_DPP_TAIL "v_cndmask_b32_e64 %[h" #p "], %[h" #p "], 0, %[mb]\n\t" \
+  "v_rcp_f32_e32 %[" #rn "], %[" #rn "]\n\t" "v_cndmask_b32_e64 %[dinv], %[dinv], %[" #rk "], %[mb]\n\t" el
+#define MZ_GJ_HINGE13(pn, el)                                                                                           \
+  MZ_GJ_CMP(mb, 13) "v_mul_f32_e64 %[h13], %[h13], -%[rj]\n\t" MZ_GJ_CMP(ma, pn) "v_cndmask_b32_e64 %[h13], %[h13], 0, %[mb]\n\t" \
+  "v_cndmask_b32_e64 %[dinv], %[dinv], %[rj], %[mb]\n\t" "s_nop 0\n\t" el
+#define MZ_GJ_OPEN "s_nop 1\n\tv_max_f32_dpp %[ri], %[h0], %[tiny] row_newbcast:0" MZ_DPP_TAIL "v_rcp_f32_e32 %[ri], %[ri]\n\t"
+#define MZ_GJ_ROOT(p) MZ_GJ_E(2, p) MZ_GJ_E(3, p) MZ_GJ_E(6, p) MZ_GJ_E(7, p) MZ_GJ_E(10, p) MZ_GJ_E(11, p)
+#define MZ_GJ_TAIL                                                           \
+  MZ_GJ_PIVOT(2, ma, MZ_GJ_CMP(mb, 3), MZ_GJ_B(2) MZ_GJ_E(3, 2) MZ_GJ_E(6, 2) MZ_GJ_E(7, 2) MZ_GJ_E(10, 2) MZ_GJ_E(11, 2))                      \
+  MZ_GJ_PIVOT(3, mb, MZ_GJ_CMP(ma, 6), MZ_GJ_B(3) MZ_GJ_E(6, 3) MZ_GJ_E(7, 3) MZ_GJ_E(10, 3) MZ_GJ_E(11, 3))                                   \
+  MZ_GJ_PIVOT(6, ma, MZ_GJ_CMP(mb, 7), MZ_GJ_B(6) MZ_GJ_E(7, 6) MZ_GJ_E(10, 6) MZ_GJ_E(11, 6))                                                \
+  MZ_GJ_PIVOT(7, mb, MZ_GJ_CMP(ma, 10), MZ_GJ_B(7) MZ_GJ_E(10, 7) MZ_GJ_E(11, 7))                                                             \
+  "s_nop 0\n\t" MZ_GJ_PIVOT(10, ma, MZ_GJ_CMP(mb, 11), MZ_GJ_B(10) MZ_GJ_E(11, 10)) "s_nop 1\n\t" MZ_GJ_PIVOT(11, mb, MZ_GJ_GAP, MZ_GJ_B(11))
+#define MZ_GJ_OPS14                                                                                                                          \
+  [b] "+v"(b), [dinv] "+v"(dinv), [h0] "+v"(H[0]), [h1] "+v"(H[1]), [h2] "+v"(H[2]), [h3] "+v"(H[3]), [h4] "+v"(H[4]), [h5] "+v"(H[5]),        \
+      [h6] "+v"(H[6]), [h7] "+v"(H[7]), [h8] "+v"(H[8]), [h9] "+v"(H[9]), [h10] "+v"(H[10]), [h11] "+v"(H[11]), [h12] "+v"(H[12]), [h13] "+v"(H[13])
+#define MZ_GJ_TMP [ri] "=&v"(ri), [rj] "=&v"(rj), [ma] "=&s"(ma), [mb] "=&s"(mb) : [tiny] "v"(tiny), [r] "v"(r)
+__device__ __forceinline__ float solve_rows(int r, float (&H)[14], float b, float& dinv) {
   dinv = 0.f;
-  const float tiny = pivot_floor();
-  pivot<0, 14, 1, 2, 3, 6, 7, 10, 11>(r, tiny, Hrow, b, dinv, mlt);
-  pivot<4, 14, 5, 2, 3, 6, 7, 10, 11>(r, tiny, Hrow, b, dinv, mlt);
-  pivot<8, 14, 9, 2, 3, 6, 7, 10, 11>(r, tiny, Hrow, b, dinv, mlt);
-  pivot<12, 14, 13, 2, 3, 6, 7, 10, 11>(r, tiny, Hrow, b, dinv, mlt);
-  pivot<1, 14, 2, 3, 6, 7, 10, 11>(r, tiny, Hrow, b, dinv, mlt);
-  pivot<5, 14, 2, 3, 6, 7, 10, 11>(r, tiny, Hrow, b, dinv, mlt);
-  pivot<9, 14, 2, 3, 6, 7, 10, 11>(r, tiny, Hrow, b, dinv, mlt);
-  pivot<13, 14, 2, 3, 6, 7, 10, 11>(r, tiny, Hrow, b, dinv, mlt);
-  pivot<2, 14, 3, 6, 7, 10, 11>(r, tiny, Hrow, b, dinv, mlt);
-  pivot<3, 14, 6, 7, 10, 11>(r, tiny, Hrow, b, dinv, mlt);
-  pivot<6, 14, 7, 10, 11>(r, tiny, Hrow, b, dinv, mlt);
-  pivot<7, 14, 10, 11>(r, tiny, Hrow, b, dinv, mlt);
-  pivot<10, 14, 11>(r, tiny, Hrow, b, dinv, mlt);
-  pivot<11, 14>(r, tiny, Hrow, b, dinv, mlt);
+  float tiny = 1e-30f, ri, rj;
+  asm("" : "+v"(tiny));
+  lanemask_t ma, mb;
+  asm(MZ_GJ_OPEN
+      MZ_GJ_HINGE(0, 4, ri, rj, MZ_GJ_B(0) MZ_GJ_E(1, 0) MZ_GJ_ROOT(0))
+      MZ_GJ_HINGE(4, 8, rj, ri, MZ_GJ_B(4) MZ_GJ_E(5, 4) MZ_GJ_ROOT(4))
+      MZ_GJ_HINGE(8, 12, ri, rj, MZ_GJ_B(8) MZ_GJ_E(9, 8) MZ_GJ_ROOT(8))
+      MZ_GJ_HINGE(12, 1, rj, ri, MZ_GJ_B(12) MZ_GJ_E(13, 12) MZ_GJ_ROOT(12))
+      MZ_GJ_HINGE(1, 5, ri, rj, MZ_GJ_B(1) MZ_GJ_ROOT(1))
+      MZ_GJ_HINGE(5, 9, rj, ri, MZ_GJ_B(5) MZ_GJ_ROOT(5))
+      MZ_GJ_HINGE(9, 13, ri, rj, MZ_GJ_B(9) MZ_GJ_ROOT(9))
+      MZ_GJ_HINGE13(2, MZ_GJ_B(13) MZ_GJ_ROOT(13))
+      MZ_GJ_TAIL
+      : MZ_GJ_OPS14, MZ_GJ_TMP);
   return b * dinv;
 }
 __device__ __forceinline__ float solve_rows(int r, float (&Hrow)[14], float b) {
-  float mlt[14], dinv;
-  return solve_rows(r, Hrow, b, mlt, dinv);
-}
-__device__ __forceinline__ float solve_rows(int r, float (&Hrow)[16], float b, float (&mlt)[16], float& dinv) {
+  float dinv;
+  return solve_rows(r, Hrow, b, dinv);
+}
+#define MZ_GJ_HUB16(p) MZ_GJ_ROOT(p) MZ_GJ_E(14, p) MZ_GJ_E(15, p)
+__device__ __forceinline__ float solve_rows(int r, float (&H)[16], float b, float& dinv) {
   dinv = 0.f;
-  const float tiny = pivot_floor();
-  pivot<0, 16, 1, 2, 3, 6, 7, 10, 11, 14, 15>(r, tiny, Hrow, b, dinv, mlt);
-  pivot<4, 16, 5, 2, 3, 6, 7, 10, 11, 14, 15>(r, tiny, Hrow, b, dinv, mlt);
-  pivot<8, 16, 9, 2, 3, 6, 7, 10, 11, 14, 15>(r, tiny, Hrow, b, dinv, mlt);
-  pivot<12, 16, 13, 2, 3, 6, 7, 10, 11, 14, 15>(r, tiny, Hrow, b, dinv, mlt);
-  pivot<1, 16, 2, 3, 6, 7, 10, 11, 14, 15>(r, tiny, Hrow, b, dinv, mlt);
-  pivot<5, 16, 2, 3, 6, 7, 10, 11, 14, 15>(r, tiny, Hrow, b, dinv, mlt);
-  pivot<9, 16, 2, 3, 6, 7, 10, 11, 14, 15>(r, tiny, Hrow, b, dinv, mlt);
-  pivot<13, 16, 2, 3, 6, 7, 10, 11, 14, 15>(r, tiny, Hrow, b, dinv, mlt);
-  pivot<14, 16, 15, 2, 3, 6, 7, 10, 11>(r, tiny, Hrow, b, dinv, mlt);
-  pivot<15, 16, 2, 3, 6, 7, 10, 11>(r, tiny, Hrow, b, dinv, mlt);
-  pivot<2, 16, 3, 6, 7, 10, 11>(r, tiny, Hrow, b, dinv, mlt);
-  pivot<3, 16, 6, 7, 10, 11>(r, tiny, Hrow, b, dinv, mlt);
-  pivot<6, 16, 7, 10, 11>(r, tiny, Hrow, b, dinv, mlt);
-  pivot<7, 16, 10, 11>(r, tiny, Hrow, b, dinv, mlt);
-  pivot<10, 16, 11>(r, tiny, Hrow, b, dinv, mlt);
-  pivot<11, 16>(r, tiny, Hrow, b, dinv, mlt);
+  float tiny = 1e-30f, ri, rj;
+  asm("" : "+v"(tiny));
+  lanemask_t ma, mb;
+  asm(MZ_GJ_OPEN
+      MZ_GJ_HINGE(0, 4, ri, rj, MZ_GJ_B(0) MZ_GJ_E(1, 0) MZ_GJ_HUB16(0))
+      MZ_GJ_HINGE(4, 8, rj, ri, MZ_GJ_B(4) MZ_GJ_E(5, 4) MZ_GJ_HUB16(4))
+      MZ_GJ_HINGE(8, 12, ri, rj, MZ_GJ_B(8) MZ_GJ_E(9, 8) MZ_GJ_HUB16(8))
+      MZ_GJ_HINGE(12, 1, rj, ri, MZ_GJ_B(12) MZ_GJ_E(13, 12) MZ_GJ_HUB16(12))
+      MZ_GJ_HINGE(1, 5, ri, rj, MZ_GJ_B(1) MZ_GJ_HUB16(1))
+      MZ_GJ_HINGE(5, 9, rj, ri, MZ_GJ_B(5) MZ_GJ_HUB16(5))
+      MZ_GJ_HINGE(9, 13, ri, rj, MZ_GJ_B(9) MZ_GJ_HUB16(9))
+      MZ_GJ_HINGE13(14, MZ_GJ_B(13) MZ_GJ_HUB16(13))
+      "s_nop 0\n\t" MZ_GJ_PIVOT(14, ma, MZ_GJ_CMP(mb, 15), MZ_GJ_B(14) MZ_GJ_E(15, 14) MZ_GJ_ROOT(14))
+      MZ_GJ_PIVOT(15, mb, MZ_GJ_CMP(ma, 2), MZ_GJ_B(15) MZ_GJ_ROOT(15))
+      MZ_GJ_TAIL
+      : MZ_GJ_OPS14, [h14] "+v"(H[14]), [h15] "+v"(H[15]), MZ_GJ_TMP);
   return b * dinv;
 }
-
 __device__ __forceinline__ float solve_rows(int r, float (&Hrow)[16], float b) {
-  float mlt[16], dinv;
-  return solve_rows(r, Hrow, b, mlt, dinv);
-}
-template <int P>
-__device__ __forceinline__ void repivot(float m, float& b) { elim<P>(m, b); }
+  float dinv;
+  return solve_rows(r, Hrow, b, dinv);
+}
+#define MZ_RP(p) "s_nop 1\n\tv_fmac_f32_dpp %[b], %[b], %[h" #p "] row_newbcast:" #p MZ_DPP_TAIL
+#define MZ_RP_LEGS MZ_RP(0) MZ_RP(4) MZ_RP(8) MZ_RP(12) MZ_RP(1) MZ_RP(5) MZ_RP(9) MZ_RP(13)
+#define MZ_RP_ROOT MZ_RP(2) MZ_RP(3) MZ_RP(6) MZ_RP(7) MZ_RP(10) MZ_RP(11)
+#define MZ_RP_IN14                                                                                                                              \
+  [h0] "v"(mlt[0]), [h1] "v"(mlt[1]), [h2] "v"(mlt[2]), [h3] "v"(mlt[3]), [h4] "v"(mlt[4]), [h5] "v"(mlt[5]), [h6] "v"(mlt[6]), [h7] "v"(mlt[7]), \
+      [h8] "v"(mlt[8]), [h9] "v"(mlt[9]), [h10] "v"(mlt[10]), [h11] "v"(mlt[11]), [h12] "v"(mlt[12]), [h13] "v"(mlt[13])
 __device__ __forceinline__ float resolve_rows(const float (&mlt)[16], float dinv, float b) {
-  repivot<0>(mlt[0], b); repivot<4>(mlt[4], b); repivot<8>(mlt[8], b); repivot<12>(mlt[12], b);
-  repivot<1>(mlt[1], b); repivot<5>(mlt[5], b); repivot<9>(mlt[9], b); repivot<13>(mlt[13], b);
-  repivot<14>(mlt[14], b); repivot<15>(mlt[15], b);
-  repivot<2>(mlt[2], b); repivot<3>(mlt[3], b); repivot<6>(mlt[6], b); repivot<7>(mlt[7], b); repivot<10>(mlt[10], b); repivot<11>(mlt[11], b);
+  asm(MZ_RP_LEGS MZ_RP(14) MZ_RP(15) MZ_RP_ROOT : [b] "+v"(b) : MZ_RP_IN14, [h14] "v"(mlt[14]), [h15] "v"(mlt[15]));
   return b * dinv;
 }
 __device__ __forceinline__ float resolve_rows(const float (&mlt)[14], float dinv, float b) {
-  repivot<0>(mlt[0], b); repivot<4>(mlt[4], b); repivot<8>(mlt[8], b); repivot<12>(mlt[12], b);
-  repivot<1>(mlt[1], b); repivot<5>(mlt[5], b); repivot<9>(mlt[9], b); repivot<13>(mlt[13], b);
-  repivot<2>(mlt[2], b); repivot<3>(mlt[3], b); repivot<6>(mlt[6], b); repivot<7>(mlt[7], b); repivot<10>(mlt[10], b); repivot<11>(mlt[11], b);
+  asm(MZ_RP_LEGS MZ_RP_ROOT : [b] "+v"(b) : MZ_RP_IN14);
   return b * dinv;
 }
 
 #define MZ_D6_MUL(o, k) "v_mul_f32_dpp %" #o ", %[f" #k "], %[s" #k "] row_newbcast:%[q]" MZ_DPP_TAIL
 #define MZ_D6_FMA(o, k) "v_fmac_f32_dpp %" #o ", %[f" #k "], %[s" #k "] row_newbcast:%[q]" MZ_DPP_TAIL
-template <int Q>
+template <int Q, int W = 2>
 __device__ __forceinline__ float dot6_from(const float (&F)[6], const float (&S)[6]) {
   float a0, a1, a2;
-  asm("s_nop 1\n\t" MZ_D6_MUL(0, 0) MZ_D6_MUL(1, 1) MZ_D6_MUL(2, 2) MZ_D6_FMA(0, 3) MZ_D6_FMA(1, 4) MZ_D6_FMA(2, 5)
+  MZ_ASM_W(W, MZ_D6_MUL(0, 0) MZ_D6_MUL(1, 1) MZ_D6_MUL(2, 2) MZ_D6_FMA(0, 3) MZ_D6_FMA(1, 4) MZ_D6_FMA(2, 5),
       : "=&v"(a0), "=&v"(a1), "=&v"(a2)
       : [f0] "v"(F[0]), [f1] "v"(F[1]), [f2] "v"(F[2]), [f3] "v"(F[3]), [f4] "v"(F[4]), [f5] "v"(F[5]), [s0] "v"(S[0]), [s1] "v"(S[1]), [s2] "v"(S[2]),
         [s3] "v"(S[3]), [s4] "v"(S[4]), [s5] "v"(S[5]), [q] "n"(Q));
   return (a0 + a1) + a2;
+}
+#define MZ_D63_MUL(a, k) "v_mul_f32_dpp %[o" #a #k "], %[f" #a #k "], %[s" #k "] row_newbcast:%[q]" MZ_DPP_TAIL
+#define MZ_D63_FMA(a, k, k3) "v_fmac_f32_dpp %[o" #a #k "], %[f" #a #k3 "], %[s" #k3 "] row_newbcast:%[q]" MZ_DPP_TAIL
+#define MZ_D63_F(a) [f##a##0] "v"(F[a][0]), [f##a##1] "v"(F[a][1]), [f##a##2] "v"(F[a][2]), [f##a##3] "v"(F[a][3]), [f##a##4] "v"(F[a][4]), [f##a##5] "v"(F[a][5])
+#define MZ_D63_O(a) [o##a##0] "=&v"(acc[a][0]), [o##a##1] "=&v"(acc[a][1]), [o##a##2] "=&v"(acc[a][2])
+template <int Q, int W = 2>
+__device__ __forceinline__ void dot6x3_from(const float (&F)[3][6], const float (&S)[6], float (&o)[3]) {
+  float acc[3][3];
+  MZ_ASM_W(W, MZ_D63_MUL(0, 0) MZ_D63_MUL(0, 1) MZ_D63_MUL(0, 2) MZ_D63_MUL(1, 0) MZ_D63_MUL(1, 1) MZ_D63_MUL(1, 2) MZ_D63_MUL(2, 0) MZ_D63_MUL(2, 1) MZ_D63_MUL(2, 2)
+           MZ_D63_FMA(0, 0, 3) MZ_D63_FMA(0, 1, 4) MZ_D63_FMA(0, 2, 5) MZ_D63_FMA(1, 0, 3) MZ_D63_FMA(1, 1, 4) MZ_D63_FMA(1, 2, 5) MZ_D63_FMA(2, 0, 3)
+           MZ_D63_FMA(2, 1, 4) MZ_D63_FMA(2, 2, 5),
+           : MZ_D63_O(0), MZ_D63_O(1), MZ_D63_O(2)
+           : MZ_D63_F(0), MZ_D63_F(1), MZ_D63_F(2), [s0] "v"(S[0]), [s1] "v"(S[1]), [s2] "v"(S[2]), [s3] "v"(S[3]), [s4] "v"(S[4]), [s5] "v"(S[5]), [q] "n"(Q));
+#pragma unroll
+  for (int a = 0; a < 3; a++) o[a] = (acc[a][0] + acc[a][1]) + acc[a][2];
 }
 __device__ __forceinline__ float ceval(float D, float u0, float u1, float u2) {
   float r0 = u0 + u1, r1 = u0 - u1, r2 = u0 + u2, r3 = u0 - u2;
@@ -569,8 +589,10 @@
     const int mc = bcast_i<(C & 15)>(wmeta[C / 16]), lc = mc & 7, cc = (mc >> 3) & 7;
     const bool sees = C < ncon && (ishinge ? (leg == lc && (d == 0 ? cc >= 2 : cc == 3)) : (r < 12 || (NB == 1 && r >= 14 && (mc & 64) != 0)));
     const int on = -(int)sees;
-#pragma unroll
-    for (int a = 0; a < 3; a++) o[a] = __int_as_float(__float_as_int(dot6_from<(C & 15)>(wr[C / 16][a], Sax)) & on);
+    float dots[3];
+    dot6x3_from<(C & 15)>(wr[C / 16], Sax, dots);
+#pragma unroll
+    for (int a = 0; a < 3; a++) o[a] = __int_as_float(__float_as_int(dots[a]) & on);
   };
   auto own_col = [&](auto Cc, float (&o)[3]) {
     constexpr int C = decltype(Cc)::value;
@@ -763,12 +785,10 @@
     each_contact([&](auto Cc) {
       constexpr int C = decltype(Cc)::value;
       {
-        float t, t0, t1, t2;
         float jc[3];
         own_col(Cc, jc);
-        fold_t<(C & 15)>(mycg[C / 16], jc[0], jc[1], jc[2], t, t0, t1, t2);
+        const float t = fold_th<(C & 15)>(Hrow, mycg[C / 16], jc[0], jc[1], jc[2]);
         g += t; ga += fabsf(t);
-        fold_h(Hrow, jc[0], jc[1], jc[2], t0, t1, t2);
       }
     });
     if constexpr (NB == 1) {
@@ -782,14 +802,14 @@
     if (!isdof) { g = 0.f; ga = 0.f; }
     float gnorm = 0.f, anorm = 0.f;
     if (it > 0) {
-      rsum2(g * g, ga * ga, gnorm, anorm);
+      rsum2_sq(g, ga, gnorm, anorm);
       gnorm = sqrtf(gnorm); anorm = sqrtf(anorm);
       if (!done && (ant_u(cx, K).inv_scale * gnorm < ant_u(cx, K).tol || gnorm <= ant_u(cx, K).rtol * anorm)) done = true;
     }
     if (!cx.any(!done)) { cx.tick(s, 5); break; }
     cx.tick(s, 5);
-    float mlt[NR], dinv;
-    const float search = solve_rows(r, Hrow, -g, mlt, dinv);
+    float dinv;
+    const float search = solve_rows(r, Hrow, -g, dinv);
     cx.tick(s, 6);
     jdot3(search, v);
     const float ljv = lsign * search;
@@ -817,8 +837,7 @@
     if (changed) {
       Ms = matvec(Mrow, search);
       float p1, p2;
-      rsum2(search * Mx, search * Ms, p1, p2);
-      rsum2(isdof ? search * search : 0.f, isdof ? qacc * qacc : 0.f, sn, qn);
+      rsum4(search * Mx, search * Ms, isdof ? search * search : 0.f, isdof ? qacc * qacc : 0.f, p1, p2, sn, qn);
       float lo = 0.f, hi = -1.f, prev_d2 = -1.f;
       const int ls_max = it < ant_u(cx, K).ls_fast_iters ? ant_u(cx, K).ls_fast : ant_u(cx, K).ls_iter;
       for (int ls = 0; ls < ls_max; ls++) {
@@ -921,7 +940,7 @@
           if (r == 15) g2 += c1;
         }
         if (!isdof) g2 = 0.f;
-        const float corr = resolve_rows(mlt, dinv, -g2);
+        const float corr = resolve_rows(Hrow, dinv, -g2);
         if (exact && !done) qacc += corr;
       }
     }
```
